# roysubhankar/dwt-domain-adaptation

Measured on AMD Instinct MI355X. Metric: imgs_per_sec, higher is better.
Workload: dtype bf16; 1 GPU; model=resnet50-dwt-mec-3stream, global_batch=1536, seq_len=224, parallelism=dp1, per_domain_batch=512, group_size=4, whiten_mode=zca

## Files before the change

### dwt_amd/kernels/dispatch.py

```python
from __future__ import annotations

import os
import warnings

_ext = None
_tried = False


def _load():
    global _ext, _tried
    if _tried:
        return _ext
    _tried = True
    try:
        import glob
        import importlib.util
        import os.path as osp

        here = osp.dirname(__file__)
        sos = sorted(glob.glob(osp.join(here, "_dwt_hip*.so")))
        if sos:
            spec = importlib.util.spec_from_file_location("dwt_amd.kernels._dwt_hip", sos[0])
            mod = importlib.util.module_from_spec(spec)
            spec.loader.exec_module(mod)
            mod.set_norm_wide(os.environ.get("DWT_AMD_NORM_WIDE", "1") != "0")
            mod.set_dense_glds(os.environ.get("DWT_AMD_DENSE_GLDS", "1") != "0")
            _ext = mod
    except Exception as exc:
        warnings.warn(f"dwt_amd HIP extension failed to load: {exc}")
        _ext = None
    return _ext


def available() -> bool:
    import torch
    if not torch.cuda.is_available():
        return False
    return _load() is not None


def ext():
    e = _load()
    if e is None:
        raise RuntimeError(
            "dwt_amd HIP extension is not built. Run `python -m dwt_amd.kernels.build` "
            "(or the repo's __graft_entry__.build()) to compile it for gfx950."
        )
    return e


def require_or_warn(opname: str) -> None:
    if os.environ.get("DWT_AMD_ALLOW_EAGER") == "1":
        warnings.warn(f"dwt_amd: running {opname} in eager fallback (DWT_AMD_ALLOW_EAGER=1)")
        return
    raise RuntimeError(
        f"dwt_amd: op '{opname}' called on a GPU but the HIP extension is not "
        "loaded. Build it with `python -m dwt_amd.kernels.build`, or set "
        "DWT_AMD_ALLOW_EAGER=1 to debug with the eager path."
    )



def whiten_multi(x, gamma, beta, running_means, running_vars, cfg,
                 stats_acc=None):
    from . import hip_ops
    return hip_ops.whiten_multi(x, gamma, beta, running_means, running_vars,
                                cfg, stats_acc)


def batch_norm_multi(x, gamma, beta, running_means, running_vars, cfg,
                     stats_acc=None):
    from . import hip_ops
    return hip_ops.batch_norm_multi(x, gamma, beta, running_means,
                                    running_vars, cfg, stats_acc)


def mec_loss(x, y):
    from . import hip_ops
    return hip_ops.mec_loss(x, y)


def entropy_loss(x):
    from . import hip_ops
    return hip_ops.entropy_loss(x)


def ce_loss(x, target):
    from . import hip_ops
    return hip_ops.ce_loss(x, target)
```

### dwt_amd/kernels/hip_ops.py

```python
from __future__ import annotations

import warnings
import torch

from . import dispatch
from ..ops.functional import _dist_world

_GEN_G_MAX = 32
_warned = set()


def _whiten_layout(x, c, g):
    if x.dim() == 4 and x.is_contiguous(memory_format=torch.channels_last) \
            and not x.is_contiguous():
        if whiten_cl_supported(c, g):
            return "cl"
    return "nchw"


def whiten_cl_supported(c, g):
    if c % 64 == 0 and (c <= 256 or c % 256 == 0) and g in (2, 4):
        gw = min(c, 256) // g
        return gw > 0 and 256 % gw == 0
    return False


def bn_cl_supported(c):
    if c % 4 != 0 or (c > 1024 and c % 1024 != 0):
        return False
    nch = min(c, 1024) // 4
    return 256 % nch == 0


def _bn_layout(x, c):
    if x.dim() == 2 and x.is_contiguous() and bn_cl_supported(c):
        return "cl"
    if x.dim() == 4 and x.is_contiguous(memory_format=torch.channels_last) \
            and not x.is_contiguous() and bn_cl_supported(c):
        return "cl"
    return "nchw"


def _flat_affine(gamma, beta, c, like):
    if gamma is None:
        return False, torch.empty(0, device=like.device, dtype=like.dtype), \
            torch.empty(0, device=like.device, dtype=like.dtype)
    return True, gamma.detach().reshape(c).contiguous(), \
        beta.detach().reshape(c).contiguous()


def _ema_update(ext, rm, new_mean, rv, new_var, momentum):
    if rm.dtype == torch.float32 and rm.is_contiguous() \
            and rv.dtype == torch.float32 and rv.is_contiguous():
        ext.ema_update(rm, new_mean, rv, new_var, momentum)
    else:
        rm.mul_(1.0 - momentum).add_(
            new_mean.reshape(rm.shape).to(rm.dtype), alpha=momentum)
        rv.mul_(1.0 - momentum).add_(
            new_var.reshape(rv.shape).to(rv.dtype), alpha=momentum)


def _warn_once(key, msg):
    if key not in _warned:
        _warned.add(key)
        warnings.warn(msg)


def _allreduce(t):
    import torch.distributed as dist
    dist.all_reduce(t)
    return t


def _ext():
    return dispatch.ext()


def _f32c(t):
    return t.detach().to(torch.float32).contiguous()


def _usable_stats_acc(acc, x, layout, training, numel):
    if acc is None or not training or layout != "cl" or x.dim() != 4:
        return None
    if acc.dtype != torch.float32 or acc.device != x.device \
            or acc.numel() != numel or not acc.is_contiguous():
        return None
    return acc.detach().reshape(-1)


class _HipWhitenMulti(torch.autograd.Function):

    @staticmethod
    def forward(ctx, x, gamma, beta, running_means, running_vars, cfg,
                stats_acc=None, res=None):
        ext = _ext()
        parts = cfg["parts"]
        g = x.shape[1] // cfg["num_groups"]
        eps, momentum = cfg["eps"], cfg["momentum"]
        training, mode, relu = cfg["training"], cfg["mode"], cfg["relu"]
        track = cfg.get("track_running_stats", True)
        ns_iters = cfg.get("ns_iters", 7)
        use_batch = training or not track

        c = x.shape[1]
        layout = _whiten_layout(x, c, g)
        if layout == "nchw":
            x = x.contiguous()
        n, c, h, w = x.shape
        assert n % parts == 0,             f"batch {n} not divisible by {parts} domain branches"
        b = n // parts
        n_groups = c // g
        ng_all = parts * n_groups
        dev = x.device
        m_count = b * h * w

        has_affine, gflat, bflat = _flat_affine(gamma, beta, c, x)

        world = _dist_world()[1] if cfg.get("stats_sync") and use_batch else 1
        ctx_count = m_count * world

        out = torch.empty_like(x)
        if use_batch:
            acc = _usable_stats_acc(stats_acc, x, layout, training,
                                    ng_all * (g + g * g))
            if acc is None:
                acc = torch.zeros(ng_all * (g + g * g), device=dev, dtype=torch.float32)
                if layout == "cl":
                    ext.whiten_stats_partial_cl(x, acc, g, c, m_count, parts)
                else:
                    ext.whiten_stats_partial(x, acc, g, parts)
            if world > 1:
                _allreduce(acc)
            mean = torch.empty(parts * c, device=dev, dtype=torch.float32)
            cov = torch.empty(ng_all, g, g, device=dev, dtype=torch.float32)
            ext.whiten_stats_final(acc, mean, cov, g, ng_all, ctx_count)
        else:
            mean = torch.stack([_f32c(running_means[p]).reshape(c)
                                for p in range(parts)]).reshape(-1).contiguous()
            cov = torch.stack([_f32c(running_vars[p]).reshape(n_groups, g, g)
                               for p in range(parts)]).reshape(ng_all, g, g).contiguous()

        wmat = torch.empty(ng_all, g, g, device=dev, dtype=torch.float32)
        if mode == "chol":
            ell = torch.empty_like(wmat)
            ext.matfn_chol_fwd(cov, wmat, ell, eps)
            saved_mat = ell
        else:
            ys = torch.empty(ng_all, ns_iters, g, g, device=dev, dtype=torch.float32)
            zs = torch.empty_like(ys)
            svals = torch.empty(ng_all, device=dev, dtype=torch.float32)
            ext.matfn_ns_fwd(cov, wmat, ys, zs, svals, eps, ns_iters)
            saved_mat = (ys, zs, svals)

        if res is not None:
            assert layout == "cl"
            ext.whiten_apply_res_cl(x, mean, wmat, gflat, bflat, res, out, g,
                                    c, m_count, True, has_affine, parts)
        elif layout == "cl":
            ext.whiten_apply_cl(x, mean, wmat, gflat, bflat, out, g, c,
                                m_count, relu, has_affine, parts)
        else:
            ext.whiten_apply(x, mean, wmat, gflat, bflat, out, g, relu,
                             has_affine, parts)

        if training and track and running_means is not None:
            with torch.no_grad():
                for p in range(parts):
                    _ema_update(ext, running_means[p], mean[p * c:(p + 1) * c],
                                running_vars[p],
                                cov[p * n_groups:(p + 1) * n_groups], momentum)

        ctx.cfg = cfg
        ctx.g = g
        ctx.layout = layout
        ctx.m_count = ctx_count
        ctx.m_local = m_count
        ctx.sync_world = world
        ctx.mean = mean
        ctx.wmat = wmat
        ctx.saved_mat = saved_mat
        ctx.has_affine = has_affine
        ctx.gflat = gflat
        ctx.bflat = bflat
        ctx.save_for_backward(x, gamma, out)
        return out

    @staticmethod
    def backward(ctx, dout):
        dx, _, dgamma, dbeta = _HipWhitenMulti.run_backward(ctx, dout)
        return dx, dgamma, dbeta, None, None, None, None

    @staticmethod
    def run_backward(ctx, dout, gb=None, join=False):
        ext = _ext()
        cfg = ctx.cfg
        parts, relu, mode, eps = cfg["parts"], cfg["relu"], cfg["mode"], cfg["eps"]
        training = cfg["training"]
        track = cfg.get("track_running_stats", True)
        ns_iters = cfg.get("ns_iters", 7)
        use_batch = training or not track
        g = ctx.g
        x, gamma, out = ctx.saved_tensors
        c = x.shape[1]
        ng_all = parts * (c // g)
        dev = x.device
        layout = ctx.layout
        if layout == "cl":
            dout = dout.contiguous(memory_format=torch.channels_last)
        else:
            dout = dout.contiguous()
        mean, wmat = ctx.mean, ctx.wmat
        m_count = ctx.m_count
        m_local = ctx.m_local

        dgb = torch.zeros(parts, 2, c, device=dev, dtype=torch.float32)
        dW = torch.zeros(ng_all, g, g, device=dev, dtype=torch.float32)
        dx = torch.empty_like(x)

        gid = None
        if join:
            assert layout == "cl"
            if gb is not None:
                gb = gb.contiguous(memory_format=torch.channels_last)
            gid = torch.empty_like(x)
            ext.whiten_join_bwd_reduce_cl(x, out, dout, gb, mean, wmat,
                                          ctx.gflat, gid, dW, dgb.reshape(-1),
                                          g, c, m_local, ctx.has_affine, parts)
            dout, relu = gid, False
        elif layout == "cl":
            ext.whiten_bwd_reduce_cl(x, dout, mean, wmat, ctx.gflat, ctx.bflat,
                                     dW, dgb.reshape(-1), g, c, m_local,
                                     relu, ctx.has_affine, parts)
        else:
            ext.whiten_bwd_reduce(x, dout, out, mean, wmat, ctx.gflat, dW,
                                  dgb.reshape(-1), g, relu, ctx.has_affine,
                                  parts)

        if use_batch:
            gdb = (ctx.gflat.float().unsqueeze(0) * dgb[:, 1]) if ctx.has_affine \
                else dgb[:, 1]
            gdb = gdb.reshape(-1).contiguous()
            dW_in = dW
            if ctx.sync_world > 1:
                dW_in = _allreduce(dW.clone())
                gdb = _allreduce(gdb.clone())
            S = torch.empty(ng_all, g, g, device=dev, dtype=torch.float32)
            corr = torch.empty(parts * c, device=dev, dtype=torch.float32)
            inv_m = 1.0 / m_count
            if mode == "chol":
                ext.matfn_chol_bwd(dW_in, wmat, ctx.saved_mat, gdb, S, corr,
                                   eps, inv_m)
            else:
                ys, zs, svals = ctx.saved_mat
                ext.matfn_ns_bwd(dW_in, wmat, ys, zs, svals, gdb, S, corr,
                                 eps, inv_m, ns_iters)
        else:
            S = torch.empty(0, device=dev)
            corr = torch.empty(0, device=dev)

        if layout == "cl":
            ext.whiten_bwd_apply_cl(x, dout, mean, wmat, ctx.gflat, ctx.bflat,
                                    S, corr, dx, g, c, m_local, relu,
                                    ctx.has_affine, use_batch, parts)
        else:
            ext.whiten_bwd_apply(x, dout, out, mean, wmat, ctx.gflat, S, corr,
                                 dx, g, relu, ctx.has_affine, use_batch, parts)

        if ctx.has_affine:
            dgamma = dgb[:, 0].sum(0).reshape(gamma.shape).to(gamma.dtype)
            dbeta = dgb[:, 1].sum(0).reshape(gamma.shape).to(gamma.dtype)
        else:
            dgamma = dbeta = None
        return dx, gid, dgamma, dbeta


def join_supported(kind, x, identity, cfg):
    if x.dtype not in (torch.float32, torch.bfloat16) or x.dim() != 4:
        return False
    if identity.shape != x.shape or identity.dtype != x.dtype \
            or identity.device != x.device \
            or identity.stride() != x.stride():
        return False
    c = x.shape[1]
    if kind == "whiten":
        return _whiten_layout(x, c, c // cfg["num_groups"]) == "cl"
    return _bn_layout(x, c) == "cl"


def whiten_join(x, identity, gamma, beta, running_means, running_vars, cfg,
                stats_acc=None):
    return _HipWhitenJoin.apply(x, identity, gamma, beta, running_means,
                                running_vars, cfg, stats_acc)


def batch_norm_join(x, identity, gamma, beta, running_means, running_vars, cfg,
                    stats_acc=None):
    return _HipBatchNormJoin.apply(x, identity, gamma, beta, running_means,
                                   running_vars, cfg, stats_acc)


def whiten_multi(x, gamma, beta, running_means, running_vars, cfg,
                 stats_acc=None):
    g = x.shape[1] // cfg["num_groups"]
    if g > _GEN_G_MAX or x.dtype not in (torch.float32, torch.bfloat16):
        _warn_once(("wh", g, x.dtype),
                   f"dwt_amd: whiten_multi g={g} dtype={x.dtype} uses the "
                   "torch path (HIP kernels cover g <= 32, fp32/bf16)")
        from ..ops.functional import WhitenMulti
        return WhitenMulti.apply(x, gamma, beta, running_means, running_vars, cfg)
    return _HipWhitenMulti.apply(x, gamma, beta, running_means, running_vars,
                                 cfg, stats_acc)


class _HipBatchNormMulti(torch.autograd.Function):
    @staticmethod
    def forward(ctx, x, gamma, beta, running_means, running_vars, cfg,
                stats_acc=None, res=None):
        ext = _ext()
        parts = cfg["parts"]
        eps, momentum = cfg["eps"], cfg["momentum"]
        training, relu = cfg["training"], cfg["relu"]
        track = cfg.get("track_running_stats", True)
        use_batch = training or not track

        spatial = x.dim() == 4
        c = x.shape[1]
        layout = _bn_layout(x, c)
        if layout == "nchw" or x.dim() == 2:
            x = x.contiguous()
        n = x.shape[0]
        assert n % parts == 0,             f"batch {n} not divisible by {parts} domain branches"
        dev = x.device
        cnt = (x.numel() // parts) // c

        has_affine, gflat, bflat = _flat_affine(gamma, beta, c, x)

        world = _dist_world()[1] if cfg.get("stats_sync") and use_batch else 1
        cnt_total = cnt * world

        out = torch.empty_like(x)
        if use_batch:
            acc = _usable_stats_acc(stats_acc, x, layout, training,
                                    parts * 2 * c)
            if acc is None:
                acc = torch.zeros(parts * 2 * c, device=dev, dtype=torch.float32)
                if layout == "cl":
                    ext.bn_stats_partial_cl(x, acc, c, cnt, parts)
                else:
                    ext.bn_stats_partial(x, acc, parts)
            if world > 1:
                _allreduce(acc)
            mean = torch.empty(parts * c, device=dev, dtype=torch.float32)
            istd = torch.empty(parts * c, device=dev, dtype=torch.float32)
            var_unb = torch.empty(parts * c, device=dev, dtype=torch.float32)
            ext.bn_stats_final(acc, mean, istd, var_unb, c, parts, cnt_total,
                               eps)
            if training and track and running_means is not None:
                with torch.no_grad():
                    for p in range(parts):
                        _ema_update(ext, running_means[p],
                                    mean[p * c:(p + 1) * c], running_vars[p],
                                    var_unb[p * c:(p + 1) * c], momentum)
        else:
            mean = torch.stack([_f32c(running_means[p]).reshape(c)
                                for p in range(parts)]).reshape(-1).contiguous()
            var = torch.stack([_f32c(running_vars[p]).reshape(c)
                               for p in range(parts)]).reshape(-1)
            istd = torch.rsqrt(var + eps).contiguous()

        if res is not None:
            assert layout == "cl" and x.dim() == 4
            ext.bn_apply_res_cl(x, mean, istd, gflat, bflat, res, out, c, cnt,
                                True, has_affine, parts)
        elif layout == "cl":
            ext.bn_apply_cl(x, mean, istd, gflat, bflat, out, c, cnt, relu,
                            has_affine, parts)
        else:
            ext.bn_apply(x, mean, istd, gflat, bflat, out, relu, has_affine,
                         parts)

        ctx.cfg = cfg
        ctx.layout = layout
        ctx.cnt = cnt
        ctx.cnt_total = cnt_total
        ctx.sync_world = world
        ctx.spatial = spatial
        ctx.mean = mean
        ctx.istd = istd
        ctx.has_affine = has_affine
        ctx.gflat = gflat
        ctx.bflat = bflat
        ctx.use_batch = use_batch
        ctx.save_for_backward(x, gamma, out)
        return out

    @staticmethod
    def backward(ctx, dout):
        dx, _, dgamma, dbeta = _HipBatchNormMulti.run_backward(ctx, dout)
        return dx, dgamma, dbeta, None, None, None, None

    @staticmethod
    def run_backward(ctx, dout, gb=None, join=False):
        ext = _ext()
        cfg = ctx.cfg
        parts, relu = cfg["parts"], cfg["relu"]
        x, gamma, out = ctx.saved_tensors
        c = x.shape[1]
        dev = x.device
        layout = ctx.layout
        if layout == "cl" and x.dim() == 4:
            dout = dout.contiguous(memory_format=torch.channels_last)
        else:
            dout = dout.contiguous()
        mean, istd = ctx.mean, ctx.istd

        sums = torch.zeros(parts, 2, c, device=dev, dtype=torch.float32)
        dx = torch.empty_like(x)
        gid = None
        if join:
            assert layout == "cl"
            if gb is not None:
                gb = gb.contiguous(memory_format=torch.channels_last)
            gid = torch.empty_like(x)
            ext.bn_join_bwd_reduce_cl(x, out, dout, gb, mean, istd, gid,
                                      sums.reshape(-1), c, ctx.cnt, parts)
            dout, relu = gid, False
        elif layout == "cl":
            ext.bn_bwd_reduce_cl(x, dout, mean, istd, ctx.gflat, ctx.bflat,
                                 sums.reshape(-1), c, ctx.cnt, relu,
                                 ctx.has_affine, parts)
        else:
            ext.bn_bwd_reduce(x, dout, out, mean, istd, sums.reshape(-1), relu,
                              parts)

        apply_sums = sums.reshape(-1)
        if ctx.sync_world > 1:
            apply_sums = _allreduce(apply_sums.clone())
        if layout == "cl":
            ext.bn_bwd_apply_cl(x, dout, mean, istd, ctx.gflat, ctx.bflat,
                                apply_sums, dx, c, ctx.cnt, relu,
                                ctx.has_affine, ctx.use_batch, parts,
                                ctx.cnt_total)
        else:
            ext.bn_bwd_apply(x, dout, out, mean, istd, ctx.gflat, apply_sums,
                             dx, relu, ctx.has_affine, ctx.use_batch,
                             ctx.cnt_total, parts)

        if ctx.has_affine:
            dgamma = sums[:, 1].sum(0).reshape(gamma.shape).to(gamma.dtype)
            dbeta = sums[:, 0].sum(0).reshape(gamma.shape).to(gamma.dtype)
        else:
            dgamma = dbeta = None
        return dx, gid, dgamma, dbeta


def _join_function(name, site):

    def forward(ctx, x, identity, gamma, beta, running_means, running_vars,
                cfg, stats_acc=None):
        ctx.set_materialize_grads(False)
        res = identity.detach()
        y = site.forward(ctx, x, gamma, beta, running_means, running_vars,
                         cfg, stats_acc, res=res)
        return y, y.view_as(y)

    def backward(ctx, ga, gb):
        if ga is None and gb is None:
            return (None,) * 8
        if ga is None:
            ga, gb = gb, None
        dx, gid, dgamma, dbeta = site.run_backward(ctx, ga, gb, join=True)
        return dx, gid, dgamma, dbeta, None, None, None, None

    return type(name, (torch.autograd.Function,),
                {"__doc__": _join_function.__doc__,
                 "forward": staticmethod(forward),
                 "backward": staticmethod(backward)})


_HipWhitenJoin = _join_function("_HipWhitenJoin", _HipWhitenMulti)
_HipBatchNormJoin = _join_function("_HipBatchNormJoin", _HipBatchNormMulti)


def batch_norm_multi(x, gamma, beta, running_means, running_vars, cfg,
                     stats_acc=None):
    if x.dtype not in (torch.float32, torch.bfloat16):
        from ..ops.functional import BatchNormMulti
        return BatchNormMulti.apply(x, gamma, beta, running_means, running_vars, cfg)
    return _HipBatchNormMulti.apply(x, gamma, beta, running_means, running_vars,
                                    cfg, stats_acc)


class _HipMecLoss(torch.autograd.Function):
    @staticmethod
    def forward(ctx, x, y):
        ext = _ext()
        x32 = x.detach().to(torch.float32).contiguous()
        y32 = y.detach().to(torch.float32).contiguous()
        n, k = x32.shape
        lx = torch.empty_like(x32)
        ly = torch.empty_like(y32)
        amin = torch.empty(n, device=x.device, dtype=torch.int32)
        loss = torch.zeros(1, device=x.device, dtype=torch.float32)
        ext.mec_fwd(x32, y32, lx, ly, amin, loss)
        ctx.save_for_backward(lx, ly, amin)
        ctx.dtypes = (x.dtype, y.dtype)
        return loss[0]

    @staticmethod
    def backward(ctx, dloss):
        ext = _ext()
        lx, ly, amin = ctx.saved_tensors
        gscale = dloss.detach().to(torch.float32).reshape(1).contiguous()
        dx = torch.empty_like(lx)
        dy = torch.empty_like(ly)
        ext.mec_bwd(lx, ly, amin, gscale, dx, dy)
        return dx.to(ctx.dtypes[0]), dy.to(ctx.dtypes[1])


class _HipEntropyLoss(torch.autograd.Function):
    @staticmethod
    def forward(ctx, x):
        ext = _ext()
        x32 = x.detach().to(torch.float32).contiguous()
        n, k = x32.shape
        q = torch.empty_like(x32)
        hper = torch.empty(n, device=x.device, dtype=torch.float32)
        loss = torch.zeros(1, device=x.device, dtype=torch.float32)
        ext.entropy_fwd(x32, q, hper, loss)
        ctx.save_for_backward(q, hper)
        ctx.dtype = x.dtype
        return loss[0]

    @staticmethod
    def backward(ctx, dloss):
        ext = _ext()
        q, hper = ctx.saved_tensors
        gscale = dloss.detach().to(torch.float32).reshape(1).contiguous()
        dx = torch.empty_like(q)
        ext.entropy_bwd(q, hper, gscale, dx)
        return dx.to(ctx.dtype)


def mec_loss(x, y):
    return _HipMecLoss.apply(x, y)


def entropy_loss(x):
    return _HipEntropyLoss.apply(x)


class _HipCELoss(torch.autograd.Function):

    @staticmethod
    def forward(ctx, x, target):
        ext = _ext()
        x32 = x.detach().to(torch.float32).contiguous()
        q = torch.empty_like(x32)
        loss = torch.zeros(1, device=x.device, dtype=torch.float32)
        ext.ce_fwd(x32, target.contiguous(), q, loss)
        ctx.save_for_backward(q, target)
        ctx.dtype = x.dtype
        return loss[0]

    @staticmethod
    def backward(ctx, dloss):
        ext = _ext()
        q, target = ctx.saved_tensors
        gscale = dloss.detach().to(torch.float32).reshape(1).contiguous()
        dx = torch.empty_like(q)
        ext.ce_bwd(q, target.contiguous(), gscale, dx)
        return dx.to(ctx.dtype), None


def ce_loss(x, target):
    return _HipCELoss.apply(x, target)
```

### dwt_amd/kernels/src/dwt_kernels.hip

```cpp

#include <torch/extension.h>
#include <ATen/cuda/CUDAContext.h>
#include <hip/hip_runtime.h>

#include <cstdint>
#include <initializer_list>
#include <string>
#include <type_traits>
#include <vector>

#define DEV_INLINE __device__ __forceinline__

namespace dwt {


DEV_INLINE float ldf(const float* p) { return *p; }
DEV_INLINE float ldf(const c10::BFloat16* p) {
  unsigned short u = *reinterpret_cast<const unsigned short*>(p);
  union { unsigned int i; float f; } v;
  v.i = static_cast<unsigned int>(u) << 16;
  return v.f;
}
DEV_INLINE void stf(float* p, float v) { *p = v; }
DEV_INLINE void stf(c10::BFloat16* p, float v) {
  union { unsigned int i; float f; } u;
  u.f = v;
  unsigned int lsb = (u.i >> 16) & 1u;
  unsigned int rounded = u.i + 0x7fffu + lsb;
  *reinterpret_cast<unsigned short*>(p) = static_cast<unsigned short>(rounded >> 16);
}

template <typename T> struct VecTraits;
template <> struct VecTraits<float> {
  static constexpr int W = 4;
  DEV_INLINE static void load(const float* p, float* out) {
    const float4 v = *reinterpret_cast<const float4*>(p);
    out[0] = v.x; out[1] = v.y; out[2] = v.z; out[3] = v.w;
  }
  DEV_INLINE static void store(float* p, const float* in) {
    *reinterpret_cast<float4*>(p) = make_float4(in[0], in[1], in[2], in[3]);
  }
};
template <> struct VecTraits<c10::BFloat16> {
  static constexpr int W = 8;
  DEV_INLINE static void load(const c10::BFloat16* p, float* out) {
    const uint4 v = *reinterpret_cast<const uint4*>(p);
    const unsigned int w[4] = {v.x, v.y, v.z, v.w};
#pragma unroll
    for (int i = 0; i < 4; ++i) {
      union { unsigned int u; float f; } lo, hi;
      lo.u = (w[i] & 0xffffu) << 16;
      hi.u = w[i] & 0xffff0000u;
      out[2 * i] = lo.f;
      out[2 * i + 1] = hi.f;
    }
  }
  DEV_INLINE static void store(c10::BFloat16* p, const float* in) {
    unsigned int w[4];
#pragma unroll
    for (int i = 0; i < 4; ++i) {
      union { unsigned int u; float f; } a, b;
      a.f = in[2 * i]; b.f = in[2 * i + 1];
      unsigned int la = (a.u >> 16) & 1u, lb = (b.u >> 16) & 1u;
      unsigned int ra = (a.u + 0x7fffu + la) >> 16;
      unsigned int rb = (b.u + 0x7fffu + lb) >> 16;
      w[i] = (ra & 0xffffu) | (rb << 16);
    }
    *reinterpret_cast<uint4*>(p) = make_uint4(w[0], w[1], w[2], w[3]);
  }
};

DEV_INLINE float wave_reduce_sum(float v) {
#pragma unroll
  for (int off = 32; off > 0; off >>= 1) v += __shfl_down(v, off, 64);
  return v;
}

template <int NV, typename IdxFn>
DEV_INLINE void block_reduce_atomic(float (&vals)[NV], float* lds,
                                    float* gout, IdxFn idx) {
  const int lane = threadIdx.x & 63;
  const int wid = threadIdx.x >> 6;
  const int nwaves = blockDim.x >> 6;
#pragma unroll
  for (int k = 0; k < NV; ++k) {
    const float r = wave_reduce_sum(vals[k]);
    if (lane == 0) lds[wid * NV + k] = r;
  }
  __syncthreads();
  for (int k = threadIdx.x; k < NV; k += blockDim.x) {
    float acc = 0.f;
    for (int w = 0; w < nwaves; ++w) acc += lds[w * NV + k];
    atomicAdd(&gout[idx(k)], acc);
  }
  __syncthreads();
}


template <typename T, int G, bool VECTOR>
__global__ void whiten_stats_partial_kernel(
    const T* __restrict__ x, float* __restrict__ acc,
    int B, int C, int64_t HW, int64_t M) {
  constexpr int VW = VECTOR ? VecTraits<T>::W : 1;
  const int grp = blockIdx.y;
  const int c0 = grp * G;
  float s[G];
  float p[G][G];
#pragma unroll
  for (int i = 0; i < G; ++i) {
    s[i] = 0.f;
#pragma unroll
    for (int j = 0; j < G; ++j) p[i][j] = 0.f;
  }
  const int64_t nvec = M / VW;
  const int64_t stride = (int64_t)gridDim.x * blockDim.x;
  for (int64_t mv = (int64_t)blockIdx.x * blockDim.x + threadIdx.x; mv < nvec; mv += stride) {
    const int64_t el = mv * VW;
    const int64_t n = el / HW, hw = el - n * HW;
    const T* base = x + ((n * C + c0) * HW + hw);
    float v[G][VW];
#pragma unroll
    for (int j = 0; j < G; ++j) {
      if (VECTOR) VecTraits<T>::load(base + (int64_t)j * HW, v[j]);
      else v[j][0] = ldf(base + (int64_t)j * HW);
    }
#pragma unroll
    for (int k = 0; k < VW; ++k) {
#pragma unroll
      for (int i = 0; i < G; ++i) {
        s[i] += v[i][k];
#pragma unroll
        for (int j = 0; j <= i; ++j) p[i][j] += v[i][k] * v[j][k];
      }
    }
  }
  float* gacc = acc + (int64_t)grp * (G + G * G);
  constexpr int NTRI = G * (G + 1) / 2;
  __shared__ float red_lds[4 * (G + NTRI)];
  float vals[G + NTRI];
#pragma unroll
  for (int i = 0; i < G; ++i) vals[i] = s[i];
#pragma unroll
  for (int i = 0; i < G; ++i)
#pragma unroll
    for (int j = 0; j <= i; ++j) vals[G + i * (i + 1) / 2 + j] = p[i][j];
  block_reduce_atomic<G + NTRI>(vals, red_lds, gacc, [](int k) {
    if (k < G) return k;
    int kk = k - G, i = 0;
    while (kk > i) { kk -= (i + 1); ++i; }
    return G + i * G + kk;
  });
}

__global__ void whiten_stats_final_kernel(
    const float* __restrict__ acc, float* __restrict__ mean,
    float* __restrict__ cov, int n_groups, int g, float inv_m) {
  const int grp = blockIdx.x;
  const int i = threadIdx.x / g, j = threadIdx.x % g;
  if (i >= g) return;
  const float* gacc = acc + (int64_t)grp * (g + g * g);
  const float mi = gacc[i] * inv_m;
  const float mj = gacc[j] * inv_m;
  const float pij = (j <= i) ? gacc[g + i * g + j] : gacc[g + j * g + i];
  cov[((int64_t)grp * g + i) * g + j] = pij * inv_m - mi * mj;
  if (j == 0) mean[grp * g + i] = mi;
}


#define GEN_MT 64

template <typename T>
DEV_INLINE void gen_load_tile(const T* __restrict__ x, float* tile, int g,
                              int C, int64_t HW, int64_t m0, int64_t M,
                              const float* __restrict__ sub ) {
  for (int idx = threadIdx.x; idx < g * GEN_MT; idx += blockDim.x) {
    const int c = idx / GEN_MT;
    const int ml = idx % GEN_MT;
    const int64_t m = m0 + ml;
    float v = 0.f;
    if (m < M) {
      const int64_t n = m / HW, hw = m - n * HW;
      v = ldf(x + (n * C + c) * HW + hw);
      if (sub) v -= sub[c];
    }
    tile[c * (GEN_MT + 1) + ml] = v;
  }
}

template <typename T>
__global__ void whiten_stats_gen_kernel(
    const T* __restrict__ x, float* __restrict__ acc,
    int g, int C, int64_t HW, int64_t M) {
  __shared__ float tile[32 * (GEN_MT + 1)];
  const int grp = blockIdx.y;
  const int c0 = grp * g;
  const int ntri = g * (g + 1) / 2;
  float p[3] = {0.f, 0.f, 0.f};
  float s = 0.f;
  const int64_t stride = (int64_t)gridDim.x * GEN_MT;
  for (int64_t m0 = (int64_t)blockIdx.x * GEN_MT; m0 < M; m0 += stride) {
    gen_load_tile(x + (int64_t)c0 * HW, tile, g, C, HW, m0, M, nullptr);
    __syncthreads();
    for (int pi = 0; pi < 3; ++pi) {
      const int pr = threadIdx.x + pi * 256;
      if (pr >= ntri) break;
      int i = 0, kk = pr;
      while (kk > i) { kk -= (i + 1); ++i; }
      const float* ri = tile + i * (GEN_MT + 1);
      const float* rj = tile + kk * (GEN_MT + 1);
      float a = 0.f;
#pragma unroll 4
      for (int ml = 0; ml < GEN_MT; ++ml) a += ri[ml] * rj[ml];
      p[pi] += a;
    }
    if (threadIdx.x < (unsigned)g) {
      const float* ri = tile + threadIdx.x * (GEN_MT + 1);
      float a = 0.f;
#pragma unroll 4
      for (int ml = 0; ml < GEN_MT; ++ml) a += ri[ml];
      s += a;
    }
    __syncthreads();
  }
  float* gacc = acc + (int64_t)grp * (g + g * g);
  if (threadIdx.x < (unsigned)g) atomicAdd(&gacc[threadIdx.x], s);
  for (int pi = 0; pi < 3; ++pi) {
    const int pr = threadIdx.x + pi * 256;
    if (pr >= ntri) break;
    int i = 0, kk = pr;
    while (kk > i) { kk -= (i + 1); ++i; }
    atomicAdd(&gacc[g + i * g + kk], p[pi]);
  }
}

template <typename T>
__global__ void whiten_apply_gen_kernel(
    const T* __restrict__ x, const float* __restrict__ mean,
    const float* __restrict__ W, const T* __restrict__ gamma,
    const T* __restrict__ beta, T* __restrict__ out,
    int g, int C, int64_t HW, int64_t M, int relu, int has_affine) {
  __shared__ float tile[32 * (GEN_MT + 1)];
  __shared__ float Ws[32 * 32];
  __shared__ float ms[32], gs[32], bs[32];
  const int grp = blockIdx.y;
  const int c0 = grp * g;
  for (int e = threadIdx.x; e < g * g; e += blockDim.x)
    Ws[e] = W[(int64_t)grp * g * g + e];
  if (threadIdx.x < (unsigned)g) {
    ms[threadIdx.x] = mean[c0 + threadIdx.x];
    gs[threadIdx.x] = has_affine ? ldf(gamma + c0 + threadIdx.x) : 1.f;
    bs[threadIdx.x] = has_affine ? ldf(beta + c0 + threadIdx.x) : 0.f;
  }
  __syncthreads();
  const int64_t stride = (int64_t)gridDim.x * GEN_MT;
  const int ml = threadIdx.x % GEN_MT;
  const int cstep = blockDim.x / GEN_MT;
  for (int64_t m0 = (int64_t)blockIdx.x * GEN_MT; m0 < M; m0 += stride) {
    gen_load_tile(x + (int64_t)c0 * HW, tile, g, C, HW, m0, M, ms);
    __syncthreads();
    const int64_t m = m0 + ml;
    if (m < M) {
      const int64_t n = m / HW, hw = m - n * HW;
      for (int c = threadIdx.x / GEN_MT; c < g; c += cstep) {
        float a = 0.f;
        for (int j = 0; j < g; ++j)
          a += Ws[c * g + j] * tile[j * (GEN_MT + 1) + ml];
        a = a * gs[c] + bs[c];
        if (relu) a = fmaxf(a, 0.f);
        stf(out + ((int64_t)n * C + c0 + c) * HW + hw, a);
      }
    }
    __syncthreads();
  }
}

template <typename T>
DEV_INLINE void gen_load_dy(const T* __restrict__ dout, const T* __restrict__ outp,
                            float* tile, int g, int C, int64_t HW, int64_t m0,
                            int64_t M, int relu) {
  for (int idx = threadIdx.x; idx < g * GEN_MT; idx += blockDim.x) {
    const int c = idx / GEN_MT;
    const int ml = idx % GEN_MT;
    const int64_t m = m0 + ml;
    float v = 0.f;
    if (m < M) {
      const int64_t n = m / HW, hw = m - n * HW;
      const int64_t off = (n * C + c) * HW + hw;
      v = ldf(dout + off);
      if (relu && ldf(outp + off) <= 0.f) v = 0.f;
    }
    tile[c * (GEN_MT + 1) + ml] = v;
  }
}

template <typename T>
__global__ void whiten_bwd_reduce_gen_kernel(
    const T* __restrict__ x, const T* __restrict__ dout,
    const T* __restrict__ outp, const float* __restrict__ mean,
    const float* __restrict__ W, const T* __restrict__ gamma,
    float* __restrict__ dWacc, float* __restrict__ dgb,
    int g, int C, int64_t HW, int64_t M, int relu, int has_affine) {
  __shared__ float xt[32 * (GEN_MT + 1)];
  __shared__ float dyt[32 * (GEN_MT + 1)];
  __shared__ float ms[32];
  const int grp = blockIdx.y;
  const int c0 = grp * g;
  if (threadIdx.x < (unsigned)g) ms[threadIdx.x] = mean[c0 + threadIdx.x];
  __syncthreads();
  const int npair = g * g;
  float p[4] = {0.f, 0.f, 0.f, 0.f};
  float db = 0.f;
  const int64_t stride = (int64_t)gridDim.x * GEN_MT;
  const int64_t xoff = (int64_t)c0 * HW;
  for (int64_t m0 = (int64_t)blockIdx.x * GEN_MT; m0 < M; m0 += stride) {
    gen_load_tile(x + xoff, xt, g, C, HW, m0, M, ms);
    gen_load_dy(dout + xoff, outp + xoff, dyt, g, C, HW, m0, M, relu);
    __syncthreads();
    for (int pi = 0; pi < 4; ++pi) {
      const int pr = threadIdx.x + pi * 256;
      if (pr >= npair) break;
      const int i = pr / g, j = pr % g;
      const float* ri = dyt + i * (GEN_MT + 1);
      const float* rj = xt + j * (GEN_MT + 1);
      float a = 0.f;
#pragma unroll 4
      for (int ml = 0; ml < GEN_MT; ++ml) a += ri[ml] * rj[ml];
      p[pi] += a;
    }
    if (threadIdx.x < (unsigned)g) {
      const float* ri = dyt + threadIdx.x * (GEN_MT + 1);
      float a = 0.f;
#pragma unroll 4
      for (int ml = 0; ml < GEN_MT; ++ml) a += ri[ml];
      db += a;
    }
    __syncthreads();
  }
  if (threadIdx.x < (unsigned)g)
    atomicAdd(&dgb[C + c0 + threadIdx.x], db);
  for (int pi = 0; pi < 4; ++pi) {
    const int pr = threadIdx.x + pi * 256;
    if (pr >= npair) break;
    const int i = pr / g, j = pr % g;
    const float gm = has_affine ? ldf(gamma + c0 + i) : 1.f;
    atomicAdd(&dWacc[(int64_t)grp * g * g + pr], gm * p[pi]);
    atomicAdd(&dgb[c0 + i], W[(int64_t)grp * g * g + i * g + j] * p[pi]);
  }
}

template <typename T>
__global__ void whiten_bwd_apply_gen_kernel(
    const T* __restrict__ x, const T* __restrict__ dout,
    const T* __restrict__ outp, const float* __restrict__ mean,
    const float* __restrict__ W, const T* __restrict__ gamma,
    const float* __restrict__ S, const float* __restrict__ corr,
    T* __restrict__ dx, int g, int C, int64_t HW, int64_t M, int relu,
    int has_affine, int train_stats) {
  __shared__ float xt[32 * (GEN_MT + 1)];
  __shared__ float dyt[32 * (GEN_MT + 1)];
  __shared__ float Ws[32 * 32];
  __shared__ float Ss[32 * 32];
  __shared__ float ms[32], gs[32], cr[32];
  const int grp = blockIdx.y;
  const int c0 = grp * g;
  for (int e = threadIdx.x; e < g * g; e += blockDim.x) {
    Ws[e] = W[(int64_t)grp * g * g + e];
    Ss[e] = train_stats ? S[(int64_t)grp * g * g + e] : 0.f;
  }
  if (threadIdx.x < (unsigned)g) {
    ms[threadIdx.x] = mean[c0 + threadIdx.x];
    gs[threadIdx.x] = has_affine ? ldf(gamma + c0 + threadIdx.x) : 1.f;
    cr[threadIdx.x] = train_stats ? corr[c0 + threadIdx.x] : 0.f;
  }
  __syncthreads();
  const int64_t stride = (int64_t)gridDim.x * GEN_MT;
  const int ml = threadIdx.x % GEN_MT;
  const int cstep = blockDim.x / GEN_MT;
  const int64_t xoff = (int64_t)c0 * HW;
  for (int64_t m0 = (int64_t)blockIdx.x * GEN_MT; m0 < M; m0 += stride) {
    gen_load_tile(x + xoff, xt, g, C, HW, m0, M, ms);
    gen_load_dy(dout + xoff, outp + xoff, dyt, g, C, HW, m0, M, relu);
    __syncthreads();
    const int64_t m = m0 + ml;
    if (m < M) {
      const int64_t n = m / HW, hw = m - n * HW;
      for (int c = threadIdx.x / GEN_MT; c < g; c += cstep) {
        float a = -cr[c];
        for (int j = 0; j < g; ++j)
          a += Ws[j * g + c] * gs[j] * dyt[j * (GEN_MT + 1) + ml] +
               Ss[c * g + j] * xt[j * (GEN_MT + 1) + ml];
        stf(dx + ((int64_t)n * C + c0 + c) * HW + hw, a);
      }
    }
    __syncthreads();
  }
}


#define MATFN_MAX_G 32

__global__ void matfn_chol_fwd_kernel(
    const float* __restrict__ cov, float* __restrict__ Wout,
    float* __restrict__ Lout, int g, float eps) {
  __shared__ float A[MATFN_MAX_G * MATFN_MAX_G];
  __shared__ float Wl[MATFN_MAX_G * MATFN_MAX_G];
  const int grp = blockIdx.x;
  const int t = threadIdx.x;
  const int64_t base = (int64_t)grp * g * g;
  for (int e = t; e < g * g; e += 64) {
    const int i = e / g, j = e % g;
    A[e] = (1.f - eps) * cov[base + e] + (i == j ? eps : 0.f);
  }
  __syncthreads();
  for (int k = 0; k < g; ++k) {
    if (t == 0) A[k * g + k] = sqrtf(A[k * g + k]);
    __syncthreads();
    const float dk = A[k * g + k];
    for (int i = k + 1 + t; i < g; i += 64) A[i * g + k] /= dk;
    __syncthreads();
    for (int e = t; e < (g - k - 1) * (g - k - 1); e += 64) {
      const int jj = k + 1 + e / (g - k - 1);
      const int ii = k + 1 + e % (g - k - 1);
      if (ii >= jj) A[ii * g + jj] -= A[ii * g + k] * A[jj * g + k];
    }
    __syncthreads();
  }
  for (int c = t; c < g; c += 64) {
    for (int i = 0; i < g; ++i) {
      float v = (i == c) ? 1.f : 0.f;
      for (int j = c; j < i; ++j) v -= A[i * g + j] * Wl[j * g + c];
      Wl[i * g + c] = (i >= c) ? v / A[i * g + i] : 0.f;
    }
  }
  __syncthreads();
  for (int e = t; e < g * g; e += 64) {
    const int i = e / g, j = e % g;
    Wout[base + e] = Wl[e];
    Lout[base + e] = (i >= j) ? A[e] : 0.f;
  }
}

__global__ void matfn_chol_bwd_kernel(
    const float* __restrict__ dW, const float* __restrict__ W,
    const float* __restrict__ L, const float* __restrict__ gdb,
    float* __restrict__ S, float* __restrict__ corr,
    int g, float eps, float inv_m) {
  __shared__ float sW[MATFN_MAX_G * MATFN_MAX_G];
  __shared__ float t0[MATFN_MAX_G * MATFN_MAX_G];
  __shared__ float t1[MATFN_MAX_G * MATFN_MAX_G];
  const int grp = blockIdx.x;
  const int t = threadIdx.x;
  const int64_t base = (int64_t)grp * g * g;
  for (int e = t; e < g * g; e += 64) { sW[e] = W[base + e]; t0[e] = dW[base + e]; }
  __syncthreads();
  for (int e = t; e < g * g; e += 64) {
    const int i = e / g, j = e % g;
    float v = 0.f;
    for (int k = 0; k < g; ++k) v += sW[k * g + i] * t0[k * g + j];
    t1[e] = v;
  }
  __syncthreads();
  for (int e = t; e < g * g; e += 64) {
    const int i = e / g, j = e % g;
    float v = 0.f;
    for (int k = 0; k < g; ++k) v += t1[i * g + k] * sW[j * g + k];
    t0[e] = (i >= j) ? -v : 0.f;
  }
  __syncthreads();
  for (int e = t; e < g * g; e += 64) {
    const int i = e / g, j = e % g;
    float v = 0.f;
    for (int k = 0; k < g; ++k) v += L[base + k * g + i] * t0[k * g + j];
    t1[e] = (i > j) ? v : (i == j ? 0.5f * v : 0.f);
  }
  __syncthreads();
  for (int e = t; e < g * g; e += 64) {
    const int i = e / g, j = e % g;
    float v = 0.f;
    for (int k = 0; k < g; ++k) v += sW[k * g + i] * t1[k * g + j];
    t0[e] = v;
  }
  __syncthreads();
  for (int e = t; e < g * g; e += 64) {
    const int i = e / g, j = e % g;
    float v = 0.f;
    for (int k = 0; k < g; ++k) v += t0[i * g + k] * sW[k * g + j];
    t1[e] = v;
  }
  __syncthreads();
  const float sc = (1.f - eps) * inv_m;
  for (int e = t; e < g * g; e += 64) {
    const int i = e / g, j = e % g;
    S[base + e] = sc * (t1[i * g + j] + t1[j * g + i]);
  }
  for (int i = t; i < g; i += 64) {
    float v = 0.f;
    for (int j = 0; j < g; ++j) v += sW[j * g + i] * gdb[grp * g + j];
    corr[grp * g + i] = v * inv_m;
  }
}

__global__ void matfn_ns_fwd_kernel(
    const float* __restrict__ cov, float* __restrict__ Wout,
    float* __restrict__ ys, float* __restrict__ zs, float* __restrict__ svals,
    int g, float eps, int iters) {
  __shared__ float Y[MATFN_MAX_G * MATFN_MAX_G];
  __shared__ float Z[MATFN_MAX_G * MATFN_MAX_G];
  __shared__ float Tm[MATFN_MAX_G * MATFN_MAX_G];
  __shared__ float NY[MATFN_MAX_G * MATFN_MAX_G];
  __shared__ float NZ[MATFN_MAX_G * MATFN_MAX_G];
  __shared__ float s_sh;
  const int grp = blockIdx.x;
  const int t = threadIdx.x;
  const int64_t base = (int64_t)grp * g * g;
  for (int e = t; e < g * g; e += 64) {
    const int i = e / g, j = e % g;
    Y[e] = (1.f - eps) * cov[base + e] + (i == j ? eps : 0.f);
  }
  __syncthreads();
  if (t == 0) {
    float tr = 0.f;
    for (int i = 0; i < g; ++i) tr += Y[i * g + i];
    s_sh = fmaxf(tr, 1e-30f);
    svals[grp] = s_sh;
  }
  __syncthreads();
  const float s = s_sh;
  for (int e = t; e < g * g; e += 64) {
    Y[e] /= s;
    Z[e] = (e / g == e % g) ? 1.f : 0.f;
  }
  __syncthreads();
  for (int it = 0; it < iters; ++it) {
    float* ysave = ys + ((int64_t)grp * iters + it) * g * g;
    float* zsave = zs + ((int64_t)grp * iters + it) * g * g;
    for (int e = t; e < g * g; e += 64) {
      ysave[e] = Y[e];
      zsave[e] = Z[e];
      const int i = e / g, j = e % g;
      float v = 0.f;
      for (int k = 0; k < g; ++k) v += Z[i * g + k] * Y[k * g + j];
      Tm[e] = 0.5f * ((i == j ? 3.f : 0.f) - v);
    }
    __syncthreads();
    for (int e = t; e < g * g; e += 64) {
      const int i = e / g, j = e % g;
      float vy = 0.f, vz = 0.f;
      for (int k = 0; k < g; ++k) {
        vy += Y[i * g + k] * Tm[k * g + j];
        vz += Tm[i * g + k] * Z[k * g + j];
      }
      NY[e] = vy;
      NZ[e] = vz;
    }
    __syncthreads();
    for (int e = t; e < g * g; e += 64) { Y[e] = NY[e]; Z[e] = NZ[e]; }
    __syncthreads();
  }
  const float inv_sqrt_s = rsqrtf(s);
  for (int e = t; e < g * g; e += 64) Wout[base + e] = Z[e] * inv_sqrt_s;
}

__global__ void matfn_ns_bwd_kernel(
    const float* __restrict__ dW, const float* __restrict__ W,
    const float* __restrict__ ys, const float* __restrict__ zs,
    const float* __restrict__ svals, const float* __restrict__ gdb,
    float* __restrict__ S, float* __restrict__ corr,
    int g, float eps, float inv_m, int iters) {
  __shared__ float YB[MATFN_MAX_G * MATFN_MAX_G];
  __shared__ float ZB[MATFN_MAX_G * MATFN_MAX_G];
  __shared__ float Tm[MATFN_MAX_G * MATFN_MAX_G];
  __shared__ float TB[MATFN_MAX_G * MATFN_MAX_G];
  __shared__ float NY[MATFN_MAX_G * MATFN_MAX_G];
  __shared__ float NZ[MATFN_MAX_G * MATFN_MAX_G];
  __shared__ float red[1];
  const int grp = blockIdx.x;
  const int t = threadIdx.x;
  const int64_t base = (int64_t)grp * g * g;
  const float s = svals[grp];
  const float inv_sqrt_s = rsqrtf(s);

  float sbar_part = 0.f;
  for (int e = t; e < g * g; e += 64) {
    const float d = dW[base + e];
    ZB[e] = d * inv_sqrt_s;
    YB[e] = 0.f;
    sbar_part += d * W[base + e];
  }
  sbar_part = wave_reduce_sum(sbar_part);
  if (t == 0) red[0] = sbar_part * (-0.5f) / s;
  __syncthreads();
  float sbar = red[0];

  for (int it = iters - 1; it >= 0; --it) {
    const float* y = ys + ((int64_t)grp * iters + it) * g * g;
    const float* z = zs + ((int64_t)grp * iters + it) * g * g;
    for (int e = t; e < g * g; e += 64) {
      const int i = e / g, j = e % g;
      float v = 0.f;
      for (int k = 0; k < g; ++k) v += z[i * g + k] * y[k * g + j];
      Tm[e] = 0.5f * ((i == j ? 3.f : 0.f) - v);
    }
    __syncthreads();
    for (int e = t; e < g * g; e += 64) {
      const int i = e / g, j = e % g;
      float v = 0.f;
      for (int k = 0; k < g; ++k)
        v += y[k * g + i] * YB[k * g + j] + ZB[i * g + k] * z[j * g + k];
      TB[e] = v;
    }
    __syncthreads();
    for (int e = t; e < g * g; e += 64) {
      const int i = e / g, j = e % g;
      float vy = 0.f, vz = 0.f;
      for (int k = 0; k < g; ++k) {
        vy += YB[i * g + k] * Tm[j * g + k] - 0.5f * z[k * g + i] * TB[k * g + j];
        vz += Tm[k * g + i] * ZB[k * g + j] - 0.5f * TB[i * g + k] * y[j * g + k];
      }
      NY[e] = vy;
      NZ[e] = vz;
    }
    __syncthreads();
    for (int e = t; e < g * g; e += 64) { YB[e] = NY[e]; ZB[e] = NZ[e]; }
    __syncthreads();
  }

  const float* y0 = ys + (int64_t)grp * iters * g * g;
  float dot = 0.f;
  for (int e = t; e < g * g; e += 64) dot += YB[e] * y0[e];
  dot = wave_reduce_sum(dot);
  if (t == 0) red[0] = dot;
  __syncthreads();
  sbar -= red[0] / s;

  const float sc = (1.f - eps) * inv_m;
  for (int e = t; e < g * g; e += 64) {
    const int i = e / g, j = e % g;
    const float raw_ij = YB[i * g + j] / s + (i == j ? sbar : 0.f);
    const float raw_ji = YB[j * g + i] / s + (i == j ? sbar : 0.f);
    S[base + e] = sc * (raw_ij + raw_ji);
  }
  for (int i = t; i < g; i += 64) {
    float v = 0.f;
    for (int j = 0; j < g; ++j) v += W[base + j * g + i] * gdb[grp * g + j];
    corr[grp * g + i] = v * inv_m;
  }
}


template <typename T, int G, bool VECTOR>
__global__ void whiten_apply_kernel(
    const T* __restrict__ x, const float* __restrict__ mean,
    const float* __restrict__ W, const T* __restrict__ gamma,
    const T* __restrict__ beta, T* __restrict__ out,
    int C, int64_t HW, int relu, int has_affine) {
  constexpr int VW = VECTOR ? VecTraits<T>::W : 1;
  const int grp = blockIdx.z;
  const int n = blockIdx.y;
  const int c0 = grp * G;
  const int64_t hw0 = ((int64_t)blockIdx.x * blockDim.x + threadIdx.x) * VW;
  if (hw0 >= HW) return;

  float m[G], Wr[G][G], gm[G], bt[G];
#pragma unroll
  for (int i = 0; i < G; ++i) {
    m[i] = mean[c0 + i];
    gm[i] = has_affine ? ldf(gamma + c0 + i) : 1.f;
    bt[i] = has_affine ? ldf(beta + c0 + i) : 0.f;
#pragma unroll
    for (int j = 0; j < G; ++j) Wr[i][j] = W[((int64_t)grp * G + i) * G + j];
  }

  const T* xb = x + ((int64_t)n * C + c0) * HW + hw0;
  T* ob = out + ((int64_t)n * C + c0) * HW + hw0;
  float xv[G][VW];
  if (VECTOR) {
#pragma unroll
    for (int j = 0; j < G; ++j) VecTraits<T>::load(xb + (int64_t)j * HW, xv[j]);
  } else {
#pragma unroll
    for (int j = 0; j < G; ++j) xv[j][0] = ldf(xb + (int64_t)j * HW);
  }
#pragma unroll
  for (int j = 0; j < G; ++j)
#pragma unroll
    for (int v = 0; v < VW; ++v) xv[j][v] -= m[j];

#pragma unroll
  for (int i = 0; i < G; ++i) {
    float yv[VW];
#pragma unroll
    for (int v = 0; v < VW; ++v) {
      float a = 0.f;
#pragma unroll
      for (int j = 0; j < G; ++j) a += Wr[i][j] * xv[j][v];
      a = a * gm[i] + bt[i];
      yv[v] = relu ? fmaxf(a, 0.f) : a;
    }
    if (VECTOR) VecTraits<T>::store(ob + (int64_t)i * HW, yv);
    else stf(ob + (int64_t)i * HW, yv[0]);
  }
}


template <typename T, int G, bool VECTOR>
__global__ void whiten_bwd_reduce_kernel(
    const T* __restrict__ x, const T* __restrict__ dout,
    const T* __restrict__ out, const float* __restrict__ mean,
    const float* __restrict__ W, const T* __restrict__ gamma,
    float* __restrict__ dWacc, float* __restrict__ dgb,
    int B, int C, int64_t HW, int64_t M, int relu, int has_affine) {
  constexpr int VW = VECTOR ? VecTraits<T>::W : 1;
  const int grp = blockIdx.y;
  const int c0 = grp * G;
  float m[G], Wr[G][G], gm[G];
#pragma unroll
  for (int i = 0; i < G; ++i) {
    m[i] = mean[c0 + i];
    gm[i] = has_affine ? ldf(gamma + c0 + i) : 1.f;
#pragma unroll
    for (int j = 0; j < G; ++j) Wr[i][j] = W[((int64_t)grp * G + i) * G + j];
  }
  float dWl[G][G], dg[G], db[G];
#pragma unroll
  for (int i = 0; i < G; ++i) {
    dg[i] = 0.f; db[i] = 0.f;
#pragma unroll
    for (int j = 0; j < G; ++j) dWl[i][j] = 0.f;
  }

  const int64_t nvec = M / VW;
  const int64_t stride = (int64_t)gridDim.x * blockDim.x;
  for (int64_t mv = (int64_t)blockIdx.x * blockDim.x + threadIdx.x; mv < nvec; mv += stride) {
    const int64_t el = mv * VW;
    const int64_t n = el / HW, hw = el - n * HW;
    const int64_t off = ((int64_t)n * C + c0) * HW + hw;
    float xv[G][VW], dyv[G][VW];
#pragma unroll
    for (int j = 0; j < G; ++j) {
      if (VECTOR) {
        VecTraits<T>::load(x + off + (int64_t)j * HW, xv[j]);
        VecTraits<T>::load(dout + off + (int64_t)j * HW, dyv[j]);
        if (relu) {
          float ov[VW];
          VecTraits<T>::load(out + off + (int64_t)j * HW, ov);
#pragma unroll
          for (int v = 0; v < VW; ++v) dyv[j][v] = ov[v] > 0.f ? dyv[j][v] : 0.f;
        }
      } else {
        xv[j][0] = ldf(x + off + (int64_t)j * HW);
        float d = ldf(dout + off + (int64_t)j * HW);
        if (relu) d = ldf(out + off + (int64_t)j * HW) > 0.f ? d : 0.f;
        dyv[j][0] = d;
      }
#pragma unroll
      for (int v = 0; v < VW; ++v) xv[j][v] -= m[j];
    }
#pragma unroll
    for (int v = 0; v < VW; ++v) {
#pragma unroll
      for (int i = 0; i < G; ++i) {
        const float dy = dyv[i][v];
        db[i] += dy;
        float y0 = 0.f;
#pragma unroll
        for (int j = 0; j < G; ++j) y0 += Wr[i][j] * xv[j][v];
        dg[i] += dy * y0;
        const float dy0 = dy * gm[i];
#pragma unroll
        for (int j = 0; j < G; ++j) dWl[i][j] += dy0 * xv[j][v];
      }
    }
  }

  float* gdW = dWacc + (int64_t)grp * G * G;
  __shared__ float red_lds[4 * G * G];
  {
    float vals[2 * G];
#pragma unroll
    for (int i = 0; i < G; ++i) { vals[i] = dg[i]; vals[G + i] = db[i]; }
    block_reduce_atomic<2 * G>(vals, red_lds, dgb, [c0, C](int k) {
      return k < G ? c0 + k : C + c0 + (k - G);
    });
  }
  {
    float vals[G * G];
#pragma unroll
    for (int i = 0; i < G; ++i)
#pragma unroll
      for (int j = 0; j < G; ++j) vals[i * G + j] = dWl[i][j];
    block_reduce_atomic<G * G>(vals, red_lds, gdW, [](int k) { return k; });
  }
}


template <typename T, int G, bool VECTOR>
__global__ void whiten_bwd_apply_kernel(
    const T* __restrict__ x, const T* __restrict__ dout,
    const T* __restrict__ out, const float* __restrict__ mean,
// ... 578 lines not shown
#pragma unroll
  for (int k = 0; k < VC; ++k) {
    atomicAdd(&lacc[cb + k], a[k]);
    atomicAdd(&lacc[L.CW + cb + k], b[k]);
  }
  __syncthreads();
  for (int k = threadIdx.x; k < L.CW; k += blockDim.x) {
    atomicAdd(&acc[blockIdx.z * 1024 + k], lacc[k]);
    atomicAdd(&acc[C + blockIdx.z * 1024 + k], lacc[L.CW + k]);
  }
}

template <typename T, int VC, int R>
__global__ void bn_stats_nhwc_kernel(
    const T* __restrict__ x, float* __restrict__ acc, int C, int64_t M) {
  const int part = blockIdx.y;
  x += (int64_t)part * M * C;
  acc += (int64_t)part * 2 * C;
  const BnLanes<VC> L(C);
  float s[VC], ss[VC];
#pragma unroll
  for (int k = 0; k < VC; ++k) { s[k] = 0.f; ss[k] = 0.f; }
  for_rows<R>(L, M, [&](int64_t m, int64_t stride, auto n) {
    constexpr int N = decltype(n)::value;
    float v[N][VC];
#pragma unroll
    for (int r = 0; r < N; ++r)
      load_group<T, VC>(x + (m + r * stride) * C + L.c0, v[r]);
#pragma unroll
    for (int r = 0; r < N; ++r)
#pragma unroll
      for (int k = 0; k < VC; ++k) { s[k] += v[r][k]; ss[k] += v[r][k] * v[r][k]; }
  });
  bn_two_sum_flush(L, C, s, ss, acc);
}

template <typename T, int VC, int R, bool RES>
__global__ void bn_apply_nhwc_kernel(
    const T* __restrict__ x, const T* __restrict__ res,
    const float* __restrict__ mean,
    const float* __restrict__ istd, const T* __restrict__ gamma,
    const T* __restrict__ beta, T* __restrict__ out, int C, int64_t M,
    int relu, int has_affine) {
  const int part = blockIdx.y;
  x += (int64_t)part * M * C;
  if constexpr (RES) res += (int64_t)part * M * C;
  out += (int64_t)part * M * C;
  mean += (int64_t)part * C;
  istd += (int64_t)part * C;
  const BnLanes<VC> L(C);
  float mu[VC], is[VC], gm[VC], bt[VC];
#pragma unroll
  for (int k = 0; k < VC; ++k) {
    mu[k] = mean[L.c0 + k];
    is[k] = istd[L.c0 + k];
    gm[k] = has_affine ? ldf(gamma + L.c0 + k) : 1.f;
    bt[k] = has_affine ? ldf(beta + L.c0 + k) : 0.f;
  }
  for_rows<R>(L, M, [&](int64_t m, int64_t stride, auto n) {
    constexpr int N = decltype(n)::value;
    [[maybe_unused]] float r[N][VC];
    float v[N][VC];
#pragma unroll
    for (int i = 0; i < N; ++i) {
      load_group<T, VC>(x + (m + i * stride) * C + L.c0, v[i]);
      if constexpr (RES) load_group<T, VC>(res + (m + i * stride) * C + L.c0, r[i]);
    }
#pragma unroll
    for (int i = 0; i < N; ++i) {
#pragma unroll
      for (int k = 0; k < VC; ++k) {
        float y = (v[i][k] - mu[k]) * is[k] * gm[k] + bt[k];
        if constexpr (RES) y += r[i][k];
        v[i][k] = relu ? fmaxf(y, 0.f) : y;
      }
      store_group<T, VC>(out + (m + i * stride) * C + L.c0, v[i]);
    }
  });
}

template <typename T, int VC, int R, bool JOIN>
__global__ void bn_bwd_reduce_nhwc_kernel(
    const T* __restrict__ x, const T* __restrict__ dout,
    const T* __restrict__ y, const T* __restrict__ gb, T* __restrict__ gid,
    const float* __restrict__ mean,
    const float* __restrict__ istd, const T* __restrict__ gamma,
    const T* __restrict__ beta, float* __restrict__ sums, int C,
    int64_t M, int relu, int has_affine) {
  const int part = blockIdx.y;
  const int64_t poff = (int64_t)part * M * C;
  x += poff; dout += poff;
  if constexpr (JOIN) {
    y += poff; gid += poff;
    if (gb) gb += poff;
  }
  mean += (int64_t)part * C;
  istd += (int64_t)part * C;
  sums += (int64_t)part * 2 * C;
  const BnLanes<VC> L(C);
  float mu[VC], is[VC], gm[VC], bt[VC];
#pragma unroll
  for (int k = 0; k < VC; ++k) {
    mu[k] = mean[L.c0 + k];
    is[k] = istd[L.c0 + k];
    gm[k] = has_affine ? ldf(gamma + L.c0 + k) : 1.f;
    bt[k] = has_affine ? ldf(beta + L.c0 + k) : 0.f;
  }
  float s_dy[VC], s_dyxh[VC];
#pragma unroll
  for (int k = 0; k < VC; ++k) { s_dy[k] = 0.f; s_dyxh[k] = 0.f; }
  for_rows<R>(L, M, [&](int64_t m, int64_t stride, auto n) {
    constexpr int N = decltype(n)::value;
    [[maybe_unused]] float yv[N][VC];
    float xv[N][VC], dv[N][VC];
#pragma unroll
    for (int i = 0; i < N; ++i) {
      if constexpr (JOIN) {
        const int64_t off = (m + i * stride) * C + L.c0;
        load_group<T, VC>(x + off, xv[i]);
        load_group<T, VC>(y + off, yv[i]);
        join_sum<T, VC>(dout, gb, off, dv[i]);
      } else {
        load_group<T, VC>(x + (m + i * stride) * C + L.c0, xv[i]);
        load_group<T, VC>(dout + (m + i * stride) * C + L.c0, dv[i]);
      }
    }
#pragma unroll
    for (int i = 0; i < N; ++i) {
#pragma unroll
      for (int k = 0; k < VC; ++k) {
        if constexpr (JOIN)
          dv[i][k] = yv[i][k] > 0.f ? round_to<T>(dv[i][k]) : 0.f;
        const float xh = (xv[i][k] - mu[k]) * is[k];
        if constexpr (!JOIN) {
          if (relu && gm[k] * xh + bt[k] <= 0.f) dv[i][k] = 0.f;
        }
        s_dy[k] += dv[i][k];
        s_dyxh[k] += dv[i][k] * xh;
      }
      if constexpr (JOIN)
        store_group<T, VC>(gid + (m + i * stride) * C + L.c0, dv[i]);
    }
  });
  bn_two_sum_flush(L, C, s_dy, s_dyxh, sums);
}

template <typename T, int VC, int R>
__global__ void bn_bwd_apply_nhwc_kernel(
    const T* __restrict__ x, const T* __restrict__ dout,
    const float* __restrict__ mean,
    const float* __restrict__ istd, const T* __restrict__ gamma,
    const T* __restrict__ beta,
    const float* __restrict__ sums, T* __restrict__ dx, int C, int64_t M,
    float inv_m, int relu, int has_affine, int use_batch) {
  const int part = blockIdx.y;
  const int64_t poff = (int64_t)part * M * C;
  x += poff; dout += poff; dx += poff;
  mean += (int64_t)part * C;
  istd += (int64_t)part * C;
  sums += (int64_t)part * 2 * C;
  const BnLanes<VC> L(C);
  float mu[VC], is[VC], gm[VC], bt[VC], mdy[VC], mdyxh[VC];
#pragma unroll
  for (int k = 0; k < VC; ++k) {
    const int c = L.c0 + k;
    mu[k] = mean[c];
    is[k] = istd[c];
    gm[k] = has_affine ? ldf(gamma + c) : 1.f;
    bt[k] = has_affine ? ldf(beta + c) : 0.f;
    mdy[k] = use_batch ? sums[c] * inv_m : 0.f;
    mdyxh[k] = use_batch ? sums[C + c] * inv_m : 0.f;
  }
  for_rows<R>(L, M, [&](int64_t m, int64_t stride, auto n) {
    constexpr int N = decltype(n)::value;
    float xv[N][VC], dv[N][VC];
#pragma unroll
    for (int i = 0; i < N; ++i) {
      load_group<T, VC>(x + (m + i * stride) * C + L.c0, xv[i]);
      load_group<T, VC>(dout + (m + i * stride) * C + L.c0, dv[i]);
    }
#pragma unroll
    for (int i = 0; i < N; ++i) {
#pragma unroll
      for (int k = 0; k < VC; ++k) {
        const float xh = (xv[i][k] - mu[k]) * is[k];
        if (relu && gm[k] * xh + bt[k] <= 0.f) dv[i][k] = 0.f;
        const float dxh = dv[i][k] * gm[k];
        if (use_batch) {
          dv[i][k] = (dxh - gm[k] * mdy[k] - xh * gm[k] * mdyxh[k]) * is[k];
        } else {
          dv[i][k] = dxh * is[k];
        }
      }
      store_group<T, VC>(dx + (m + i * stride) * C + L.c0, dv[i]);
    }
  });
}


template <typename T, bool VECTOR>
__global__ void bn_stats_partial_kernel(
    const T* __restrict__ x, float* __restrict__ acc,
    int B, int C, int64_t HW, int64_t M) {
  constexpr int VW = VECTOR ? VecTraits<T>::W : 1;
  const int c = blockIdx.y;
  float s = 0.f, ss = 0.f;
  const int64_t nvec = M / VW;
  const int64_t stride = (int64_t)gridDim.x * blockDim.x;
  for (int64_t mv = (int64_t)blockIdx.x * blockDim.x + threadIdx.x; mv < nvec; mv += stride) {
    const int64_t el = mv * VW;
    const int64_t n = el / HW, hw = el - n * HW;
    const T* p = x + ((int64_t)n * C + c) * HW + hw;
    if (VECTOR) {
      float v[VW];
      VecTraits<T>::load(p, v);
#pragma unroll
      for (int k = 0; k < VW; ++k) { s += v[k]; ss += v[k] * v[k]; }
    } else {
      const float v = ldf(p);
      s += v; ss += v * v;
    }
  }
  __shared__ float red_lds[4 * 2];
  float vals[2] = {s, ss};
  block_reduce_atomic<2>(vals, red_lds, acc, [c, C](int k) {
    return k == 0 ? c : C + c;
  });
}

__global__ void bn_stats_final_kernel(
    const float* __restrict__ acc, float* __restrict__ mean,
    float* __restrict__ istd, float* __restrict__ var_unb,
    int total, int Cper, float inv_m, float unb_scale, float eps) {
  const int i = blockIdx.x * blockDim.x + threadIdx.x;
  if (i >= total) return;
  const int p = i / Cper, c = i % Cper;
  const int64_t base = (int64_t)p * 2 * Cper;
  const float mu = acc[base + c] * inv_m;
  float var = fmaxf(acc[base + Cper + c] * inv_m - mu * mu, 0.f);
  mean[i] = mu;
  istd[i] = rsqrtf(var + eps);
  var_unb[i] = var * unb_scale;
}

template <typename T, bool VECTOR>
__global__ void bn_apply_kernel(
    const T* __restrict__ x, const float* __restrict__ mean,
    const float* __restrict__ istd, const T* __restrict__ gamma,
    const T* __restrict__ beta, T* __restrict__ out,
    int C, int64_t HW, int relu, int has_affine) {
  constexpr int VW = VECTOR ? VecTraits<T>::W : 1;
  const int c = blockIdx.z;
  const int n = blockIdx.y;
  const int64_t hw0 = ((int64_t)blockIdx.x * blockDim.x + threadIdx.x) * VW;
  if (hw0 >= HW) return;
  const float mu = mean[c], is = istd[c];
  const float gm = has_affine ? ldf(gamma + c) : 1.f;
  const float bt = has_affine ? ldf(beta + c) : 0.f;
  const int64_t off = ((int64_t)n * C + c) * HW + hw0;
  float v[VW];
  if (VECTOR) VecTraits<T>::load(x + off, v);
  else v[0] = ldf(x + off);
#pragma unroll
  for (int k = 0; k < VW; ++k) {
    float y = (v[k] - mu) * is * gm + bt;
    v[k] = relu ? fmaxf(y, 0.f) : y;
  }
  if (VECTOR) VecTraits<T>::store(out + off, v);
  else stf(out + off, v[0]);
}

template <typename T, bool VECTOR>
__global__ void bn_bwd_reduce_kernel(
    const T* __restrict__ x, const T* __restrict__ dout,
    const T* __restrict__ out, const float* __restrict__ mean,
    const float* __restrict__ istd, float* __restrict__ sums,
    int B, int C, int64_t HW, int64_t M, int relu) {
  constexpr int VW = VECTOR ? VecTraits<T>::W : 1;
  const int c = blockIdx.y;
  const float mu = mean[c], is = istd[c];
  float s_dy = 0.f, s_dyxh = 0.f;
  const int64_t nvec = M / VW;
  const int64_t stride = (int64_t)gridDim.x * blockDim.x;
  for (int64_t mv = (int64_t)blockIdx.x * blockDim.x + threadIdx.x; mv < nvec; mv += stride) {
    const int64_t el = mv * VW;
    const int64_t n = el / HW, hw = el - n * HW;
    const int64_t off = ((int64_t)n * C + c) * HW + hw;
    float xv[VW], dv[VW];
    if (VECTOR) {
      VecTraits<T>::load(x + off, xv);
      VecTraits<T>::load(dout + off, dv);
      if (relu) {
        float ov[VW];
        VecTraits<T>::load(out + off, ov);
#pragma unroll
        for (int k = 0; k < VW; ++k) dv[k] = ov[k] > 0.f ? dv[k] : 0.f;
      }
    } else {
      xv[0] = ldf(x + off);
      dv[0] = ldf(dout + off);
      if (relu) dv[0] = ldf(out + off) > 0.f ? dv[0] : 0.f;
    }
#pragma unroll
    for (int k = 0; k < VW; ++k) {
      s_dy += dv[k];
      s_dyxh += dv[k] * (xv[k] - mu) * is;
    }
  }
  __shared__ float red_lds[4 * 2];
  float vals[2] = {s_dy, s_dyxh};
  block_reduce_atomic<2>(vals, red_lds, sums, [c, C](int k) {
    return k == 0 ? c : C + c;
  });
}

template <typename T, bool VECTOR>
__global__ void bn_bwd_apply_kernel(
    const T* __restrict__ x, const T* __restrict__ dout,
    const T* __restrict__ out, const float* __restrict__ mean,
    const float* __restrict__ istd, const T* __restrict__ gamma,
    const float* __restrict__ sums, T* __restrict__ dx,
    int C, int64_t HW, float inv_m, int relu, int has_affine, int use_batch) {
  constexpr int VW = VECTOR ? VecTraits<T>::W : 1;
  const int c = blockIdx.z;
  const int n = blockIdx.y;
  const int64_t hw0 = ((int64_t)blockIdx.x * blockDim.x + threadIdx.x) * VW;
  if (hw0 >= HW) return;
  const float mu = mean[c], is = istd[c];
  const float gm = has_affine ? ldf(gamma + c) : 1.f;
  const float m_dy = sums[c] * inv_m;
  const float m_dyxh = sums[C + c] * inv_m;
  const int64_t off = ((int64_t)n * C + c) * HW + hw0;
  float xv[VW], dv[VW];
  if (VECTOR) {
    VecTraits<T>::load(x + off, xv);
    VecTraits<T>::load(dout + off, dv);
    if (relu) {
      float ov[VW];
      VecTraits<T>::load(out + off, ov);
#pragma unroll
      for (int k = 0; k < VW; ++k) dv[k] = ov[k] > 0.f ? dv[k] : 0.f;
    }
  } else {
    xv[0] = ldf(x + off);
    dv[0] = ldf(dout + off);
    if (relu) dv[0] = ldf(out + off) > 0.f ? dv[0] : 0.f;
  }
#pragma unroll
  for (int k = 0; k < VW; ++k) {
    const float dxh = dv[k] * gm;
    float r;
    if (use_batch) {
      const float xh = (xv[k] - mu) * is;
      r = (dxh - gm * m_dy - xh * gm * m_dyxh) * is;
    } else {
      r = dxh * is;
    }
    dv[k] = r;
  }
  if (VECTOR) VecTraits<T>::store(dx + off, dv);
  else stf(dx + off, dv[0]);
}


__global__ void ema_update_kernel(float* __restrict__ rm,
                                  const float* __restrict__ a, int64_t n1,
                                  float* __restrict__ rv,
                                  const float* __restrict__ b, int64_t n2,
                                  float momentum) {
  const int64_t i = (int64_t)blockIdx.x * blockDim.x + threadIdx.x;
  if (i < n1) {
    rm[i] = (1.f - momentum) * rm[i] + momentum * a[i];
  } else if (i < n1 + n2) {
    const int64_t j = i - n1;
    rv[j] = (1.f - momentum) * rv[j] + momentum * b[j];
  }
}


template <typename T>
__global__ void maxpool_nhwc_fwd_kernel(
    const T* __restrict__ x, T* __restrict__ out, uint8_t* __restrict__ idx,
    int C, int H, int W, int P, int Q, int KS, int stride, int pad,
    int64_t total) {
  const int64_t i = (int64_t)blockIdx.x * blockDim.x + threadIdx.x;
  if (i >= total) return;
  const int c = i % C;
  int64_t r = i / C;
  const int q = r % Q; r /= Q;
  const int p = r % P; r /= P;
  const int n = (int)r;
  float best = -INFINITY;
  int bidx = 0;
  for (int kh = 0; kh < KS; ++kh) {
    const int h = p * stride - pad + kh;
    if (h < 0 || h >= H) continue;
    for (int kw = 0; kw < KS; ++kw) {
      const int w = q * stride - pad + kw;
      if (w < 0 || w >= W) continue;
      const float v = ldf(x + (((int64_t)n * H + h) * W + w) * C + c);
      if (v > best) { best = v; bidx = kh * KS + kw; }
    }
  }
  stf(out + i, best);
  idx[i] = (uint8_t)bidx;
}

template <typename T>
__global__ void maxpool_nhwc_bwd_kernel(
    const T* __restrict__ dout, const uint8_t* __restrict__ idx,
    T* __restrict__ dx, int C, int H, int W, int P, int Q, int KS, int stride,
    int pad, int64_t total_in) {
  const int64_t i = (int64_t)blockIdx.x * blockDim.x + threadIdx.x;
  if (i >= total_in) return;
  const int c = i % C;
  int64_t r = i / C;
  const int w = r % W; r /= W;
  const int h = r % H; r /= H;
  const int n = (int)r;
  float acc = 0.f;
  const int pmin = max(0, (h + pad - KS + stride) / stride);
  const int pmax = min(P - 1, (h + pad) / stride);
  const int qmin = max(0, (w + pad - KS + stride) / stride);
  const int qmax = min(Q - 1, (w + pad) / stride);
  for (int p = pmin; p <= pmax; ++p) {
    const int kh = h - (p * stride - pad);
    if (kh < 0 || kh >= KS) continue;
    for (int q = qmin; q <= qmax; ++q) {
      const int kw = w - (q * stride - pad);
      if (kw < 0 || kw >= KS) continue;
      const int64_t o = (((int64_t)n * P + p) * Q + q) * C + c;
      if (idx[o] == (uint8_t)(kh * KS + kw)) acc += ldf(dout + o);
    }
  }
  stf(dx + i, acc);
}

template <typename T, int VC>
__global__ void maxpool_nhwc_fwd_vec_kernel(
    const T* __restrict__ x, T* __restrict__ out, uint8_t* __restrict__ idx,
    int C, int H, int W, int P, int Q, int KS, int stride, int pad,
    int64_t total_chunks) {
  const int64_t i = (int64_t)blockIdx.x * blockDim.x + threadIdx.x;
  if (i >= total_chunks) return;
  const int nc = C / VC;
  const int c0 = (int)(i % nc) * VC;
  int64_t r = i / nc;
  const int q = r % Q; r /= Q;
  const int p = r % P; r /= P;
  const int n = (int)r;
  float best[VC];
  uint8_t bidx[VC];
#pragma unroll
  for (int k = 0; k < VC; ++k) { best[k] = -INFINITY; bidx[k] = 0; }
  for (int kh = 0; kh < KS; ++kh) {
    const int h = p * stride - pad + kh;
    if (h < 0 || h >= H) continue;
    for (int kw = 0; kw < KS; ++kw) {
      const int w = q * stride - pad + kw;
      if (w < 0 || w >= W) continue;
      float v[VC];
      load_group<T, VC>(x + (((int64_t)n * H + h) * W + w) * C + c0, v);
      const uint8_t wi = (uint8_t)(kh * KS + kw);
#pragma unroll
      for (int k = 0; k < VC; ++k)
        if (v[k] > best[k]) { best[k] = v[k]; bidx[k] = wi; }
    }
  }
  const int64_t o = (((int64_t)n * P + p) * Q + q) * C + c0;
  store_group<T, VC>(out + o, best);
#pragma unroll
  for (int k = 0; k < VC; ++k) idx[o + k] = bidx[k];
}

template <typename T, int VC>
__global__ void maxpool_nhwc_bwd_vec_kernel(
    const T* __restrict__ dout, const uint8_t* __restrict__ idx,
    T* __restrict__ dx, int C, int H, int W, int P, int Q, int KS, int stride,
    int pad, int64_t total_chunks) {
  const int64_t i = (int64_t)blockIdx.x * blockDim.x + threadIdx.x;
  if (i >= total_chunks) return;
  const int nc = C / VC;
  const int c0 = (int)(i % nc) * VC;
  int64_t r = i / nc;
  const int w = r % W; r /= W;
  const int h = r % H; r /= H;
  const int n = (int)r;
  float acc[VC];
#pragma unroll
  for (int k = 0; k < VC; ++k) acc[k] = 0.f;
  const int pmin = max(0, (h + pad - KS + stride) / stride);
  const int pmax = min(P - 1, (h + pad) / stride);
  const int qmin = max(0, (w + pad - KS + stride) / stride);
  const int qmax = min(Q - 1, (w + pad) / stride);
  for (int p = pmin; p <= pmax; ++p) {
    const int kh = h - (p * stride - pad);
    if (kh < 0 || kh >= KS) continue;
    for (int q = qmin; q <= qmax; ++q) {
      const int kw = w - (q * stride - pad);
      if (kw < 0 || kw >= KS) continue;
      const int64_t o = (((int64_t)n * P + p) * Q + q) * C + c0;
      const uint8_t wi = (uint8_t)(kh * KS + kw);
      float dv[VC];
      load_group<T, VC>(dout + o, dv);
#pragma unroll
      for (int k = 0; k < VC; ++k)
        if (idx[o + k] == wi) acc[k] += dv[k];
    }
  }
  store_group<T, VC>(dx + (((int64_t)n * H + h) * W + w) * C + c0, acc);
}

template <typename T>
__global__ void gap_nhwc_fwd_kernel(const T* __restrict__ x,
                                    T* __restrict__ out, int C, int64_t HW,
                                    int N) {
  const int n = blockIdx.y;
  const int c = blockIdx.x * 64 + (threadIdx.x & 63);
  if (c >= C) return;
  const T* base = x + (int64_t)n * HW * C + c;
  float s = 0.f;
  for (int64_t m = 0; m < HW; ++m) s += ldf(base + m * C);
  stf(out + (int64_t)n * C + c, s / (float)HW);
}

template <typename T>
__global__ void gap_nhwc_bwd_kernel(const T* __restrict__ dout,
                                    T* __restrict__ dx, int C, int64_t HW,
// ... 151 lines not shown
}

__global__ void mec_bwd_kernel(
    const float* __restrict__ lx, const float* __restrict__ ly,
    const int* __restrict__ amin, const float* __restrict__ gscale,
    float* __restrict__ dx, float* __restrict__ dy, int N, int K) {
  const int64_t i = (int64_t)blockIdx.x * blockDim.x + threadIdx.x;
  if (i >= (int64_t)N * K) return;
  const int row = i / K, k = i % K;
  const float sc = gscale[0] / (2.f * N);
  const float oh = (k == amin[row]) ? 1.f : 0.f;
  dx[i] = (__expf(lx[i]) - oh) * sc;
  dy[i] = (__expf(ly[i]) - oh) * sc;
}

__global__ void entropy_fwd_kernel(
    const float* __restrict__ x, float* __restrict__ q,
    float* __restrict__ hper, float* __restrict__ loss, int N, int K) {
  const int row = blockIdx.x * (blockDim.x / 64) + (threadIdx.x / 64);
  const int lane = threadIdx.x & 63;
  if (row >= N) return;
  const float* xr = x + (int64_t)row * K;
  float mx = -INFINITY;
  for (int k = lane; k < K; k += 64) mx = fmaxf(mx, xr[k]);
#pragma unroll
  for (int off = 32; off > 0; off >>= 1) mx = fmaxf(mx, __shfl_down(mx, off, 64));
  mx = __shfl(mx, 0, 64);
  float s = 0.f;
  for (int k = lane; k < K; k += 64) s += __expf(xr[k] - mx);
  s = wave_reduce_sum(s);
  s = __shfl(s, 0, 64);
  const float lse = mx + __logf(s);
  float h = 0.f;
  for (int k = lane; k < K; k += 64) {
    const float qq = xr[k] - lse;
    q[(int64_t)row * K + k] = qq;
    h -= __expf(qq) * qq;
  }
  h = wave_reduce_sum(h);
  if (lane == 0) {
    hper[row] = h;
    atomicAdd(loss, h / N);
  }
}

__global__ void ce_fwd_kernel(
    const float* __restrict__ x, const int64_t* __restrict__ target,
    float* __restrict__ q, float* __restrict__ loss, int N, int K) {
  const int row = blockIdx.x * (blockDim.x / 64) + (threadIdx.x / 64);
  const int lane = threadIdx.x & 63;
  if (row >= N) return;
  const float* xr = x + (int64_t)row * K;
  float mx = -INFINITY;
  for (int k = lane; k < K; k += 64) mx = fmaxf(mx, xr[k]);
#pragma unroll
  for (int off = 32; off > 0; off >>= 1) mx = fmaxf(mx, __shfl_down(mx, off, 64));
  mx = __shfl(mx, 0, 64);
  float ssum = 0.f;
  for (int k = lane; k < K; k += 64) ssum += __expf(xr[k] - mx);
  ssum = wave_reduce_sum(ssum);
  ssum = __shfl(ssum, 0, 64);
  const float lse = mx + __logf(ssum);
  for (int k = lane; k < K; k += 64) q[(int64_t)row * K + k] = xr[k] - lse;
  if (lane == 0) atomicAdd(loss, (lse - xr[target[row]]) / N);
}

__global__ void ce_bwd_kernel(
    const float* __restrict__ q, const int64_t* __restrict__ target,
    const float* __restrict__ gscale, float* __restrict__ dx, int N, int K) {
  const int64_t i = (int64_t)blockIdx.x * blockDim.x + threadIdx.x;
  if (i >= (int64_t)N * K) return;
  const int row = i / K, k = i % K;
  const float oh = (k == (int)target[row]) ? 1.f : 0.f;
  dx[i] = (__expf(q[i]) - oh) * gscale[0] / N;
}

__global__ void entropy_bwd_kernel(
    const float* __restrict__ q, const float* __restrict__ hper,
    const float* __restrict__ gscale, float* __restrict__ dx, int N, int K) {
  const int64_t i = (int64_t)blockIdx.x * blockDim.x + threadIdx.x;
  if (i >= (int64_t)N * K) return;
  const int row = i / K;
  const float p = __expf(q[i]);
  dx[i] = -p * (q[i] + hper[row]) * gscale[0] / N;
}

}


namespace {

using torch::Tensor;

inline hipStream_t cur_stream() {
  return at::cuda::getCurrentCUDAStream().stream();
}

inline int64_t elementwise_blocks(int64_t work, int threads) {
  return std::max<int64_t>(1, (work + threads - 1) / threads);
}

inline int64_t reduce_blocks(int64_t work_per_group, int threads, int vec,
                             int64_t n_groups) {
  const int64_t want = (work_per_group + (int64_t)threads * vec - 1) /
                       ((int64_t)threads * vec);
  const int64_t cap = std::max<int64_t>(1, 4096 / std::max<int64_t>(n_groups, 1));
  return std::min<int64_t>(std::max<int64_t>(want, 1), cap);
}

#define DISPATCH_FT(TENSOR, NAME, ...)                                         \
  [&] {                                                                        \
    switch ((TENSOR).scalar_type()) {                                          \
      case at::ScalarType::Float: {                                            \
        using scalar_t = float;                                                \
        return __VA_ARGS__();                                                  \
      }                                                                        \
      case at::ScalarType::BFloat16: {                                         \
        using scalar_t = c10::BFloat16;                                        \
        return __VA_ARGS__();                                                  \
      }                                                                        \
      default:                                                                 \
        TORCH_CHECK(false, NAME, ": unsupported dtype ", (TENSOR).scalar_type()); \
    }                                                                          \
  }()

template <typename T>
inline T* opt_ptr(const Tensor& t, bool present) {
  return present ? t.data_ptr<T>() : nullptr;
}
template <typename T>
inline T* opt_ptr(const c10::optional<Tensor>& t) {
  return t.has_value() ? t->data_ptr<T>() : nullptr;
}


void whiten_stats_final(Tensor acc, Tensor mean, Tensor cov, int64_t g,
                        int64_t n_groups, int64_t count) {
  const int fin_threads = std::min<int64_t>(g * g, 1024);
  hipLaunchKernelGGL(dwt::whiten_stats_final_kernel, dim3(n_groups),
                     dim3(fin_threads), 0, cur_stream(), acc.data_ptr<float>(),
                     mean.data_ptr<float>(), cov.data_ptr<float>(),
                     (int)n_groups, (int)g, 1.0f / (float)count);
}

void bn_stats_final(Tensor acc, Tensor mean, Tensor istd, Tensor var_unb,
                    int64_t C, int64_t parts, int64_t count, double eps) {
  const float unb = count > 1 ? (float)count / (float)(count - 1) : 1.f;
  const int total = parts * C;
  hipLaunchKernelGGL(dwt::bn_stats_final_kernel, dim3((total + 255) / 256),
                     dim3(256), 0, cur_stream(), acc.data_ptr<float>(),
                     mean.data_ptr<float>(), istd.data_ptr<float>(),
                     var_unb.data_ptr<float>(), total, (int)C,
                     1.0f / (float)count, unb, (float)eps);
}

struct NchwParts {
  const char* name;
  int64_t parts, HW, M, numel;
  int B, C;

  NchwParts(const char* name_, const Tensor& x, int64_t parts_,
            std::initializer_list<Tensor> streamed = {})
      : name(name_), parts(parts_) {
    TORCH_CHECK(x.is_contiguous() && (x.dim() == 4 || x.dim() == 2), name,
                ": x must be contiguous (N, C, H, W) or (N, C)");
    TORCH_CHECK(parts > 0 && x.size(0) % parts == 0, name, ": batch ",
                x.size(0), " does not split into ", parts, " branches");
    for (const Tensor& t : streamed)
      TORCH_CHECK(t.scalar_type() == x.scalar_type() &&
                      t.numel() == x.numel() && t.is_contiguous(),
                  name, ": dtype, size or layout mismatch with x");
    B = x.size(0) / parts;
    C = x.size(1);
    HW = x.dim() == 4 ? x.size(2) * x.size(3) : 1;
    M = (int64_t)B * HW;
    numel = M * C;
  }
  int groups(int64_t g) const {
    TORCH_CHECK(g > 0 && C % g == 0, name, ": group size ", g,
                " does not divide C = ", C);
    return C / g;
  }
  void stacked(std::initializer_list<std::pair<Tensor, int64_t>> ops) const {
    for (const auto& [t, per] : ops)
      TORCH_CHECK(t.numel() == parts * per, name, ": a stacked operand has ",
                  t.numel(), " elements, expected ", parts * per);
  }
};

template <typename T>
struct NchwBranch {
  const NchwParts& d;
  int64_t p;
  T* operator()(const Tensor& t) const { return t.data_ptr<T>() + p * d.numel; }
  float* operator()(const Tensor& t, int64_t per) const {
    return t.data_ptr<float>() + p * per;
  }
};

template <typename T>
bool can_vectorize(const T* p, int64_t HW) {
  return HW % dwt::VecTraits<T>::W == 0 &&
         reinterpret_cast<uintptr_t>(p) % 16 == 0;
}

template <typename F>
inline void vec_launch(bool vec, F&& f) {
  if (vec) f(std::true_type{});
  else f(std::false_type{});
}

template <typename F, typename Gen>
inline void whiten_nchw_launch(const char* name, int64_t g, bool vec, F&& f,
                               Gen&& gen) {
  auto blocked = [&](auto gconst) {
    vec_launch(vec, [&](auto vconst) { f(gconst, vconst); });
  };
  switch (g) {
    case 2: blocked(std::integral_constant<int, 2>{}); break;
    case 4: blocked(std::integral_constant<int, 4>{}); break;
    case 8: blocked(std::integral_constant<int, 8>{}); break;
    default:
      TORCH_CHECK(g <= 32, name, ": unsupported group size ", g);
      gen();
  }
}

inline dim3 nchw_reduce_grid(int64_t M, int per_block, int vw, int rows) {
  return dim3(reduce_blocks(M, per_block, vw, rows), rows);
}
inline dim3 nchw_elem_grid(int64_t HW, int vw, int B, int rows) {
  return dim3((HW + (int64_t)256 * vw - 1) / ((int64_t)256 * vw), B, rows);
}

void whiten_stats_partial(Tensor x, Tensor acc, int64_t g, int64_t parts) {
  const NchwParts d("whiten_stats", x, parts);
  const int n_groups = d.groups(g);
  const int64_t n_acc = n_groups * (g + g * g);
  d.stacked({{acc, n_acc}});
  DISPATCH_FT(x, "whiten_stats", [&] {
    constexpr int VW = dwt::VecTraits<scalar_t>::W;
    for (int64_t p = 0; p < parts; ++p) {
      const NchwBranch<scalar_t> at{d, p};
      const bool vec = g <= 4 && can_vectorize(at(x), d.HW) && d.M % VW == 0;
      whiten_nchw_launch(d.name, g, vec, [&](auto gconst, auto vconst) {
        constexpr int G = decltype(gconst)::value;
        constexpr bool V = decltype(vconst)::value;
        hipLaunchKernelGGL((dwt::whiten_stats_partial_kernel<scalar_t, G, V>),
                           nchw_reduce_grid(d.M, 256, V ? VW : 1, n_groups),
                           dim3(256), 0, cur_stream(), at(x), at(acc, n_acc),
                           d.B, d.C, d.HW, d.M);
      }, [&] {
        hipLaunchKernelGGL((dwt::whiten_stats_gen_kernel<scalar_t>),
                           nchw_reduce_grid(d.M, 64, 1, n_groups), dim3(256), 0,
                           cur_stream(), at(x), at(acc, n_acc), (int)g, d.C,
                           d.HW, d.M);
      });
    }
  });
}

void whiten_apply(Tensor x, Tensor mean, Tensor W, Tensor gamma, Tensor beta,
                  Tensor out, int64_t g, bool relu, bool has_affine,
                  int64_t parts) {
  const NchwParts d("whiten_apply", x, parts, {out});
  const int n_groups = d.groups(g);
  const int64_t n_w = n_groups * g * g;
  d.stacked({{mean, d.C}, {W, n_w}});
  DISPATCH_FT(x, "whiten_apply", [&] {
    constexpr int VW = dwt::VecTraits<scalar_t>::W;
    const scalar_t* gp = opt_ptr<scalar_t>(gamma, has_affine);
    const scalar_t* bp = opt_ptr<scalar_t>(beta, has_affine);
    for (int64_t p = 0; p < parts; ++p) {
      const NchwBranch<scalar_t> at{d, p};
      const bool vec = can_vectorize(at(x), d.HW) && can_vectorize(at(out), d.HW);
      auto launch = [&](auto kernel, dim3 grid, auto... dims) {
        hipLaunchKernelGGL(kernel, grid, dim3(256), 0, cur_stream(), at(x),
                           at(mean, d.C), at(W, n_w), gp, bp, at(out), dims...,
                           relu ? 1 : 0, has_affine ? 1 : 0);
      };
      whiten_nchw_launch(d.name, g, vec, [&](auto gconst, auto vconst) {
        constexpr int G = decltype(gconst)::value;
        constexpr bool V = decltype(vconst)::value;
        launch(dwt::whiten_apply_kernel<scalar_t, G, V>,
               nchw_elem_grid(d.HW, V ? VW : 1, d.B, n_groups), d.C, d.HW);
      }, [&] {
        launch(dwt::whiten_apply_gen_kernel<scalar_t>,
               nchw_reduce_grid(d.M, 64, 1, n_groups), (int)g, d.C, d.HW, d.M);
      });
    }
  });
}

void whiten_bwd_reduce(Tensor x, Tensor dout, Tensor out, Tensor mean, Tensor W,
                       Tensor gamma, Tensor dWacc, Tensor dgb, int64_t g,
                       bool relu, bool has_affine, int64_t parts) {
  const NchwParts d("whiten_bwd_reduce", x, parts, {dout, out});
  const int n_groups = d.groups(g);
  const int64_t n_w = n_groups * g * g;
  d.stacked({{mean, d.C}, {W, n_w}, {dWacc, n_w}, {dgb, 2 * d.C}});
  DISPATCH_FT(x, "whiten_bwd_reduce", [&] {
    constexpr int VW = dwt::VecTraits<scalar_t>::W;
    const scalar_t* gp = opt_ptr<scalar_t>(gamma, has_affine);
    for (int64_t p = 0; p < parts; ++p) {
      const NchwBranch<scalar_t> at{d, p};
      const bool vec = g <= 4 && can_vectorize(at(x), d.HW) &&
// ... 352 lines not shown
            has_affine ? 1 : 0);
      });
    });
  });
}

void whiten_join_bwd_reduce_cl(Tensor x, Tensor y, Tensor ga,
                               c10::optional<Tensor> gb, Tensor mean, Tensor W,
                               Tensor gamma, Tensor gid, Tensor dWacc,
                               Tensor dgb, int64_t g, int64_t C, int64_t M,
                               bool has_affine, int64_t parts) {
  check_join_args("whiten_join_bwd_reduce_cl", x, y, ga, gb, gid,
                  parts * M * C);
  DISPATCH_FT(x, "whiten_join_bwd_reduce_cl", [&] {
    DWT_SWITCH_G(g, {
      const bool wide = whiten_wide(
          g, C, {raw_ptr(x), raw_ptr(y), raw_ptr(ga), raw_ptr(gb), raw_ptr(gid)});
      whiten_launch<scalar_t, G, kWhitenJoinReduceWide>(wide, [&](auto w) {
        constexpr bool WIDE = decltype(w)::value;
        hipLaunchKernelGGL(
            (dwt::whiten_bwd_reduce_nhwc_kernel<scalar_t, G, WIDE, true>),
            whiten_grid(kReduce, G, C, M, parts, WIDE), dim3(256), 0,
            cur_stream(), x.data_ptr<scalar_t>(), ga.data_ptr<scalar_t>(),
            y.data_ptr<scalar_t>(), opt_ptr<scalar_t>(gb),
            gid.data_ptr<scalar_t>(), mean.data_ptr<float>(),
            W.data_ptr<float>(), opt_ptr<scalar_t>(gamma, has_affine),
            (const scalar_t*)nullptr, dWacc.data_ptr<float>(),
            dgb.data_ptr<float>(), (int)C, M, 0, has_affine ? 1 : 0);
      });
    });
  });
}

void whiten_bwd_apply_cl(Tensor x, Tensor dout, Tensor mean,
                         Tensor W, Tensor gamma, Tensor beta,
                         Tensor S, Tensor corr,
                         Tensor dx, int64_t g, int64_t C, int64_t M, bool relu,
                         bool has_affine, bool train_stats, int64_t parts) {
  DISPATCH_FT(x, "whiten_bwd_apply_cl", [&] {
    DWT_SWITCH_G(g, {
      const bool wide =
          whiten_wide(g, C, {raw_ptr(x), raw_ptr(dout), raw_ptr(dx)});
      whiten_launch<scalar_t, G, kWhitenBwdApplyWide>(wide, [&](auto w) {
        constexpr bool WIDE = decltype(w)::value;
        hipLaunchKernelGGL(
            (dwt::whiten_bwd_apply_nhwc_kernel<scalar_t, G, WIDE>),
            whiten_grid(kElem, G, C, M, parts, WIDE), dim3(256), 0,
            cur_stream(), x.data_ptr<scalar_t>(), dout.data_ptr<scalar_t>(),
            mean.data_ptr<float>(), W.data_ptr<float>(),
            opt_ptr<scalar_t>(gamma, has_affine),
            opt_ptr<scalar_t>(beta, has_affine), S.data_ptr<float>(),
            corr.data_ptr<float>(), dx.data_ptr<scalar_t>(), (int)C, M,
            relu ? 1 : 0, has_affine ? 1 : 0, train_stats ? 1 : 0);
      });
    });
  });
}

void bn_stats_partial_cl(Tensor x, Tensor acc, int64_t C, int64_t M,
                         int64_t parts) {
  DISPATCH_FT(x, "bn_stats_cl", [&] {
    bn_launch<scalar_t, kBnStatsRows, kBnStatsWide>(bn_wide(C, {raw_ptr(x)}), [&](auto vc, auto rows) {
      constexpr int VC = decltype(vc)::value, R = decltype(rows)::value;
      hipLaunchKernelGGL((dwt::bn_stats_nhwc_kernel<scalar_t, VC, R>),
                         bn_grid(kReduce, C, M, parts, VC, R), dim3(256), 0,
                         cur_stream(), x.data_ptr<scalar_t>(),
                         acc.data_ptr<float>(), (int)C, M);
    });
  });
}

void bn_apply_res_cl(Tensor x, Tensor mean, Tensor istd, Tensor gamma,
                     Tensor beta, c10::optional<Tensor> res, Tensor out,
                     int64_t C, int64_t M, bool relu, bool has_affine,
                     int64_t parts) {
  TORCH_CHECK(!res.has_value() || (res->scalar_type() == x.scalar_type() &&
                                   res->numel() == x.numel()),
              "bn_apply_res_cl: res mismatch");
  DISPATCH_FT(x, "bn_apply_cl", [&] {
    const bool wide = bn_wide(C, {raw_ptr(x), raw_ptr(res), raw_ptr(out)});
    auto launch = [&](auto with_res, auto wide_rows) {
      constexpr bool RES = decltype(with_res)::value;
      constexpr bool kInUse = RES ? kBnApplyResWide : kBnApplyWide;
      bn_launch<scalar_t, decltype(wide_rows)::value, kInUse>(wide, [&](auto vc, auto rows) {
        constexpr int VC = decltype(vc)::value, R = decltype(rows)::value;
        hipLaunchKernelGGL((dwt::bn_apply_nhwc_kernel<scalar_t, VC, R, RES>),
                           bn_grid(kElem, C, M, parts, VC, R), dim3(256), 0,
                           cur_stream(), x.data_ptr<scalar_t>(),
                           opt_ptr<scalar_t>(res), mean.data_ptr<float>(),
                           istd.data_ptr<float>(),
                           opt_ptr<scalar_t>(gamma, has_affine),
                           opt_ptr<scalar_t>(beta, has_affine),
                           out.data_ptr<scalar_t>(), (int)C, M, relu ? 1 : 0,
                           has_affine ? 1 : 0);
      });
    };
    if (res.has_value())
      launch(std::true_type{}, std::integral_constant<int, kBnApplyResRows>{});
    else
      launch(std::false_type{}, std::integral_constant<int, kBnApplyRows>{});
  });
}

void bn_apply_cl(Tensor x, Tensor mean, Tensor istd, Tensor gamma, Tensor beta,
                 Tensor out, int64_t C, int64_t M, bool relu, bool has_affine,
                 int64_t parts) {
  bn_apply_res_cl(x, mean, istd, gamma, beta, c10::nullopt, out, C, M, relu,
                  has_affine, parts);
}

void bn_bwd_reduce_cl(Tensor x, Tensor dout, Tensor mean,
                      Tensor istd, Tensor gamma, Tensor beta,
                      Tensor sums, int64_t C, int64_t M,
                      bool relu, bool has_affine, int64_t parts) {
  DISPATCH_FT(x, "bn_bwd_reduce_cl", [&] {
    const bool wide = bn_wide(C, {raw_ptr(x), raw_ptr(dout)});
    bn_launch<scalar_t, kBnReduceRows, kBnReduceWide>(wide, [&](auto vc, auto rows) {
      constexpr int VC = decltype(vc)::value, R = decltype(rows)::value;
      hipLaunchKernelGGL(
          (dwt::bn_bwd_reduce_nhwc_kernel<scalar_t, VC, R, false>),
          bn_grid(kReduce, C, M, parts, VC, R), dim3(256), 0, cur_stream(),
          x.data_ptr<scalar_t>(), dout.data_ptr<scalar_t>(),
          (const scalar_t*)nullptr, (const scalar_t*)nullptr,
          (scalar_t*)nullptr, mean.data_ptr<float>(), istd.data_ptr<float>(),
          opt_ptr<scalar_t>(gamma, has_affine),
          opt_ptr<scalar_t>(beta, has_affine), sums.data_ptr<float>(), (int)C,
          M, relu ? 1 : 0, has_affine ? 1 : 0);
    });
  });
}

void bn_join_bwd_reduce_cl(Tensor x, Tensor y, Tensor ga,
                           c10::optional<Tensor> gb, Tensor mean, Tensor istd,
                           Tensor gid, Tensor sums, int64_t C, int64_t M,
                           int64_t parts) {
  check_join_args("bn_join_bwd_reduce_cl", x, y, ga, gb, gid, parts * M * C);
  DISPATCH_FT(x, "bn_join_bwd_reduce_cl", [&] {
    const bool wide = bn_wide(
        C, {raw_ptr(x), raw_ptr(y), raw_ptr(ga), raw_ptr(gb), raw_ptr(gid)});
    bn_launch<scalar_t, kBnReduceRows, kBnJoinReduceWide>(wide, [&](auto vc, auto rows) {
      constexpr int VC = decltype(vc)::value, R = decltype(rows)::value;
      hipLaunchKernelGGL(
          (dwt::bn_bwd_reduce_nhwc_kernel<scalar_t, VC, R, true>),
          bn_grid(kReduce, C, M, parts, VC, R), dim3(256), 0, cur_stream(),
          x.data_ptr<scalar_t>(), ga.data_ptr<scalar_t>(),
          y.data_ptr<scalar_t>(), opt_ptr<scalar_t>(gb),
          gid.data_ptr<scalar_t>(), mean.data_ptr<float>(),
          istd.data_ptr<float>(), (const scalar_t*)nullptr,
          (const scalar_t*)nullptr, sums.data_ptr<float>(), (int)C, M, 0, 0);
    });
  });
}

void bn_bwd_apply_cl(Tensor x, Tensor dout, Tensor mean,
                     Tensor istd, Tensor gamma, Tensor beta,
                     Tensor sums, Tensor dx,
                     int64_t C, int64_t M, bool relu, bool has_affine,
                     bool use_batch, int64_t parts, int64_t count) {
  DISPATCH_FT(x, "bn_bwd_apply_cl", [&] {
    const bool wide = bn_wide(C, {raw_ptr(x), raw_ptr(dout), raw_ptr(dx)});
    bn_launch<scalar_t, kBnBwdApplyRows, kBnBwdApplyWide>(wide, [&](auto vc, auto rows) {
      constexpr int VC = decltype(vc)::value, R = decltype(rows)::value;
      hipLaunchKernelGGL((dwt::bn_bwd_apply_nhwc_kernel<scalar_t, VC, R>),
                         bn_grid(kElem, C, M, parts, VC, R), dim3(256), 0,
                         cur_stream(), x.data_ptr<scalar_t>(),
                         dout.data_ptr<scalar_t>(), mean.data_ptr<float>(),
                         istd.data_ptr<float>(),
                         opt_ptr<scalar_t>(gamma, has_affine),
                         opt_ptr<scalar_t>(beta, has_affine),
                         sums.data_ptr<float>(), dx.data_ptr<scalar_t>(),
                         (int)C, M, 1.0f / (float)count, relu ? 1 : 0,
                         has_affine ? 1 : 0, use_batch ? 1 : 0);
    });
  });
}

void matfn_chol_fwd(Tensor cov, Tensor W, Tensor L, double eps) {
  const int n_groups = cov.size(0);
  const int g = cov.size(1);
  TORCH_CHECK(g <= MATFN_MAX_G, "group size too large for matfn");
  hipLaunchKernelGGL(dwt::matfn_chol_fwd_kernel, dim3(n_groups), dim3(64), 0,
                     cur_stream(), cov.data_ptr<float>(), W.data_ptr<float>(),
                     L.data_ptr<float>(), g, (float)eps);
}

void matfn_chol_bwd(Tensor dW, Tensor W, Tensor L, Tensor gdb, Tensor S,
                    Tensor corr, double eps, double inv_m) {
  const int n_groups = W.size(0);
  const int g = W.size(1);
  hipLaunchKernelGGL(dwt::matfn_chol_bwd_kernel, dim3(n_groups), dim3(64), 0,
                     cur_stream(), dW.data_ptr<float>(), W.data_ptr<float>(),
                     L.data_ptr<float>(), gdb.data_ptr<float>(),
                     S.data_ptr<float>(), corr.data_ptr<float>(), g, (float)eps,
                     (float)inv_m);
}

void matfn_ns_fwd(Tensor cov, Tensor W, Tensor ys, Tensor zs, Tensor svals,
                  double eps, int64_t iters) {
  const int n_groups = cov.size(0);
  const int g = cov.size(1);
  TORCH_CHECK(g <= MATFN_MAX_G, "group size too large for matfn");
  hipLaunchKernelGGL(dwt::matfn_ns_fwd_kernel, dim3(n_groups), dim3(64), 0,
                     cur_stream(), cov.data_ptr<float>(), W.data_ptr<float>(),
                     ys.data_ptr<float>(), zs.data_ptr<float>(),
                     svals.data_ptr<float>(), g, (float)eps, (int)iters);
}

void matfn_ns_bwd(Tensor dW, Tensor W, Tensor ys, Tensor zs, Tensor svals,
                  Tensor gdb, Tensor S, Tensor corr, double eps, double inv_m,
                  int64_t iters) {
  const int n_groups = W.size(0);
  const int g = W.size(1);
  hipLaunchKernelGGL(dwt::matfn_ns_bwd_kernel, dim3(n_groups), dim3(64), 0,
                     cur_stream(), dW.data_ptr<float>(), W.data_ptr<float>(),
                     ys.data_ptr<float>(), zs.data_ptr<float>(),
                     svals.data_ptr<float>(), gdb.data_ptr<float>(),
                     S.data_ptr<float>(), corr.data_ptr<float>(), g, (float)eps,
                     (float)inv_m, (int)iters);
}

void maxpool_cl_fwd(Tensor x, Tensor out, Tensor idx, int64_t C, int64_t H,
                    int64_t W, int64_t P, int64_t Q, int64_t KS,
                    int64_t stride, int64_t pad) {
  const int64_t total = out.numel();
  DISPATCH_FT(x, "maxpool_cl_fwd", [&] {
    constexpr int VC = dwt::VecTraits<scalar_t>::W;
    if (C % VC == 0) {
      const int64_t chunks = total / VC;
      hipLaunchKernelGGL((dwt::maxpool_nhwc_fwd_vec_kernel<scalar_t, VC>),
                         dim3(elementwise_blocks(chunks, 256)), dim3(256), 0,
                         cur_stream(), x.data_ptr<scalar_t>(),
                         out.data_ptr<scalar_t>(), idx.data_ptr<uint8_t>(),
                         (int)C, (int)H, (int)W, (int)P, (int)Q, (int)KS,
                         (int)stride, (int)pad, chunks);
    } else {
      hipLaunchKernelGGL((dwt::maxpool_nhwc_fwd_kernel<scalar_t>),
                         dim3(elementwise_blocks(total, 256)), dim3(256), 0,
                         cur_stream(), x.data_ptr<scalar_t>(),
                         out.data_ptr<scalar_t>(), idx.data_ptr<uint8_t>(),
                         (int)C, (int)H, (int)W, (int)P, (int)Q, (int)KS,
                         (int)stride, (int)pad, total);
    }
  });
}

void maxpool_cl_bwd(Tensor dout, Tensor idx, Tensor dx, int64_t C, int64_t H,
                    int64_t W, int64_t P, int64_t Q, int64_t KS,
                    int64_t stride, int64_t pad) {
  const int64_t total_in = dx.numel();
  DISPATCH_FT(dout, "maxpool_cl_bwd", [&] {
    constexpr int VC = dwt::VecTraits<scalar_t>::W;
    if (C % VC == 0) {
      const int64_t chunks = total_in / VC;
      hipLaunchKernelGGL((dwt::maxpool_nhwc_bwd_vec_kernel<scalar_t, VC>),
                         dim3(elementwise_blocks(chunks, 256)), dim3(256), 0,
                         cur_stream(), dout.data_ptr<scalar_t>(),
                         idx.data_ptr<uint8_t>(), dx.data_ptr<scalar_t>(),
                         (int)C, (int)H, (int)W, (int)P, (int)Q, (int)KS,
                         (int)stride, (int)pad, chunks);
    } else {
      hipLaunchKernelGGL((dwt::maxpool_nhwc_bwd_kernel<scalar_t>),
                         dim3(elementwise_blocks(total_in, 256)), dim3(256), 0,
                         cur_stream(), dout.data_ptr<scalar_t>(),
                         idx.data_ptr<uint8_t>(), dx.data_ptr<scalar_t>(),
                         (int)C, (int)H, (int)W, (int)P, (int)Q, (int)KS,
                         (int)stride, (int)pad, total_in);
    }
  });
}

void gap_cl_fwd(Tensor x, Tensor out, int64_t C, int64_t HW, int64_t N) {
  DISPATCH_FT(x, "gap_cl_fwd", [&] {
    dim3 grid((C + 63) / 64, N);
    hipLaunchKernelGGL((dwt::gap_nhwc_fwd_kernel<scalar_t>), grid, dim3(64), 0,
                       cur_stream(), x.data_ptr<scalar_t>(),
                       out.data_ptr<scalar_t>(), (int)C, HW, (int)N);
  });
}

void gap_cl_bwd(Tensor dout, Tensor dx, int64_t C, int64_t HW) {
  const int64_t total = dx.numel();
  DISPATCH_FT(dout, "gap_cl_bwd", [&] {
    hipLaunchKernelGGL((dwt::gap_nhwc_bwd_kernel<scalar_t>),
                       dim3(elementwise_blocks(total, 256)), dim3(256), 0,
                       cur_stream(), dout.data_ptr<scalar_t>(),
                       dx.data_ptr<scalar_t>(), (int)C, HW, total);
  });
}

void add_relu_fwd(Tensor a, Tensor b, Tensor out) {
  const int64_t n = a.numel();
  DISPATCH_FT(a, "add_relu_fwd", [&] {
    constexpr int VW = dwt::VecTraits<scalar_t>::W;
    const bool vec = (n % VW == 0) &&
        (reinterpret_cast<uintptr_t>(a.data_ptr()) % 16 == 0) &&
        (reinterpret_cast<uintptr_t>(b.data_ptr()) % 16 == 0);
    const int64_t per = vec ? (n + 256 * VW - 1) / (256 * VW)
                            : (n + 255) / 256;
    if (vec)
      hipLaunchKernelGGL((dwt::add_relu_fwd_kernel<scalar_t, true>), dim3(per),
                         dim3(256), 0, cur_stream(), a.data_ptr<scalar_t>(),
                         b.data_ptr<scalar_t>(), out.data_ptr<scalar_t>(), n);
    else
      hipLaunchKernelGGL((dwt::add_relu_fwd_kernel<scalar_t, false>), dim3(per),
                         dim3(256), 0, cur_stream(), a.data_ptr<scalar_t>(),
                         b.data_ptr<scalar_t>(), out.data_ptr<scalar_t>(), n);
  });
}

void add_relu_bwd(Tensor dout, Tensor out, Tensor din) {
  const int64_t n = dout.numel();
  DISPATCH_FT(dout, "add_relu_bwd", [&] {
    constexpr int VW = dwt::VecTraits<scalar_t>::W;
    const bool vec = (n % VW == 0) &&
        (reinterpret_cast<uintptr_t>(dout.data_ptr()) % 16 == 0);
    const int64_t per = vec ? (n + 256 * VW - 1) / (256 * VW)
                            : (n + 255) / 256;
    if (vec)
      hipLaunchKernelGGL((dwt::add_relu_bwd_kernel<scalar_t, true>), dim3(per),
                         dim3(256), 0, cur_stream(), dout.data_ptr<scalar_t>(),
                         out.data_ptr<scalar_t>(), din.data_ptr<scalar_t>(), n);
    else
      hipLaunchKernelGGL((dwt::add_relu_bwd_kernel<scalar_t, false>), dim3(per),
                         dim3(256), 0, cur_stream(), dout.data_ptr<scalar_t>(),
                         out.data_ptr<scalar_t>(), din.data_ptr<scalar_t>(), n);
  });
}

void fused_sgd(Tensor desc, int64_t n_chunks, double lr, double momentum,
               double wd, bool bf16_params, bool master, bool zero_grad,
               bool first_step) {
  auto lp = [&](auto tconst, auto mconst) {
    using T = typename decltype(tconst)::type;
    constexpr bool M = decltype(mconst)::value;
    hipLaunchKernelGGL((dwt::sgd_kernel<T, M>), dim3(n_chunks), dim3(256), 0,
                       cur_stream(), desc.data_ptr<int64_t>(), (float)lr,
                       (float)momentum, (float)wd, zero_grad ? 1 : 0,
                       first_step ? 1 : 0);
  };
  struct FT { using type = float; };
  struct BT { using type = c10::BFloat16; };
  if (bf16_params) {
    if (master) lp(BT{}, std::true_type{}); else lp(BT{}, std::false_type{});
  } else {
    if (master) lp(FT{}, std::true_type{}); else lp(FT{}, std::false_type{});
  }
}

void fused_adam(Tensor desc, int64_t n_chunks, double lr, double beta1,
                double beta2, double eps, double wd, double bc1, double bc2,
                bool bf16_params, bool master, bool zero_grad) {
  auto lp = [&](auto tconst, auto mconst) {
    using T = typename decltype(tconst)::type;
    constexpr bool M = decltype(mconst)::value;
    hipLaunchKernelGGL((dwt::adam_kernel<T, M>), dim3(n_chunks), dim3(256), 0,
                       cur_stream(), desc.data_ptr<int64_t>(), (float)lr,
                       (float)beta1, (float)beta2, (float)eps, (float)wd,
                       (float)bc1, (float)bc2, zero_grad ? 1 : 0);
  };
  struct FT { using type = float; };
  struct BT { using type = c10::BFloat16; };
  if (bf16_params) {
    if (master) lp(BT{}, std::true_type{}); else lp(BT{}, std::false_type{});
  } else {
    if (master) lp(FT{}, std::true_type{}); else lp(FT{}, std::false_type{});
  }
}

void ema_update(Tensor rm, Tensor a, Tensor rv, Tensor b, double momentum) {
  const int64_t n1 = rm.numel(), n2 = rv.numel();
  hipLaunchKernelGGL(dwt::ema_update_kernel,
                     dim3(elementwise_blocks(n1 + n2, 256)), dim3(256), 0,
                     cur_stream(), rm.data_ptr<float>(), a.data_ptr<float>(),
                     n1, rv.data_ptr<float>(), b.data_ptr<float>(), n2,
                     (float)momentum);
}


void mec_fwd(Tensor x, Tensor y, Tensor lx, Tensor ly, Tensor amin, Tensor loss) {
  const int N = x.size(0), K = x.size(1);
  const int rows_per_block = 4;
  hipLaunchKernelGGL(dwt::mec_fwd_kernel,
                     dim3((N + rows_per_block - 1) / rows_per_block),
                     dim3(rows_per_block * 64), 0, cur_stream(),
                     x.data_ptr<float>(), y.data_ptr<float>(),
                     lx.data_ptr<float>(), ly.data_ptr<float>(),
                     amin.data_ptr<int>(), loss.data_ptr<float>(), N, K);
}

void mec_bwd(Tensor lx, Tensor ly, Tensor amin, Tensor gscale, Tensor dx, Tensor dy) {
  const int N = lx.size(0), K = lx.size(1);
  const int64_t total = (int64_t)N * K;
  hipLaunchKernelGGL(dwt::mec_bwd_kernel, dim3(elementwise_blocks(total, 256)),
                     dim3(256), 0, cur_stream(), lx.data_ptr<float>(),
                     ly.data_ptr<float>(), amin.data_ptr<int>(),
                     gscale.data_ptr<float>(), dx.data_ptr<float>(),
                     dy.data_ptr<float>(), N, K);
}

void entropy_fwd(Tensor x, Tensor q, Tensor hper, Tensor loss) {
  const int N = x.size(0), K = x.size(1);
  const int rows_per_block = 4;
  hipLaunchKernelGGL(dwt::entropy_fwd_kernel,
                     dim3((N + rows_per_block - 1) / rows_per_block),
                     dim3(rows_per_block * 64), 0, cur_stream(),
                     x.data_ptr<float>(), q.data_ptr<float>(),
                     hper.data_ptr<float>(), loss.data_ptr<float>(), N, K);
}

void ce_fwd(Tensor x, Tensor target, Tensor q, Tensor loss) {
  const int N = x.size(0), K = x.size(1);
  const int rows_per_block = 4;
  hipLaunchKernelGGL(dwt::ce_fwd_kernel,
                     dim3((N + rows_per_block - 1) / rows_per_block),
                     dim3(rows_per_block * 64), 0, cur_stream(),
                     x.data_ptr<float>(), target.data_ptr<int64_t>(),
                     q.data_ptr<float>(), loss.data_ptr<float>(), N, K);
}

void ce_bwd(Tensor q, Tensor target, Tensor gscale, Tensor dx) {
  const int N = q.size(0), K = q.size(1);
  hipLaunchKernelGGL(dwt::ce_bwd_kernel,
                     dim3(elementwise_blocks((int64_t)N * K, 256)), dim3(256),
                     0, cur_stream(), q.data_ptr<float>(),
                     target.data_ptr<int64_t>(), gscale.data_ptr<float>(),
                     dx.data_ptr<float>(), N, K);
}

void entropy_bwd(Tensor q, Tensor hper, Tensor gscale, Tensor dx) {
  const int N = q.size(0), K = q.size(1);
  const int64_t total = (int64_t)N * K;
  hipLaunchKernelGGL(dwt::entropy_bwd_kernel,
                     dim3(elementwise_blocks(total, 256)), dim3(256), 0,
                     cur_stream(), q.data_ptr<float>(), hper.data_ptr<float>(),
                     gscale.data_ptr<float>(), dx.data_ptr<float>(), N, K);
}

}

void mfma_gemm(torch::Tensor a, torch::Tensor bt, torch::Tensor bias,
               torch::Tensor out, bool relu, bool has_bias);
void mfma_conv2d_fwd(torch::Tensor x, torch::Tensor wgt, torch::Tensor bias,
                     torch::Tensor out, int64_t N, int64_t H, int64_t W,
                     int64_t Cin, int64_t P, int64_t Q, int64_t Cout,
                     int64_t KH, int64_t KW, int64_t stride, int64_t pad,
                     bool relu, bool has_bias);
void mfma_conv2d_fwd_fused(torch::Tensor x, torch::Tensor wgt,
                           torch::Tensor bias, torch::Tensor res,
                           torch::Tensor out, int64_t N, int64_t H, int64_t W,
                           int64_t Cin, int64_t P, int64_t Q, int64_t Cout,
                           int64_t KH, int64_t KW, int64_t stride, int64_t pad,
                           bool relu, bool has_res);
void conv1x1_stats(torch::Tensor x, torch::Tensor wgt, torch::Tensor out,
                   torch::Tensor acc, int64_t kind, int64_t g, int64_t parts,
                   int64_t max_workgroups);
void mfma_conv2d_dgrad(torch::Tensor dy, torch::Tensor wd, torch::Tensor dx,
                       int64_t N, int64_t H, int64_t W, int64_t Cin,
                       int64_t P, int64_t Q, int64_t Cdy, int64_t KH,
                       int64_t KW, int64_t stride, int64_t pad);
void mfma_conv2d_wgrad(torch::Tensor dy, torch::Tensor x, torch::Tensor dw,
                       torch::Tensor ws, int64_t N, int64_t H, int64_t W,
                       int64_t Cin, int64_t P, int64_t Q, int64_t Cout,
                       int64_t KH, int64_t KW, int64_t stride, int64_t pad);
void set_dense_glds(bool on);
bool dense_glds_selected();
int64_t dense_glds_launches();

void assemble_views(torch::Tensor images, torch::Tensor src_index,
                    torch::Tensor top, torch::Tensor left, torch::Tensor flags,
                    torch::Tensor inv_affine, torch::Tensor out,
                    std::vector<double> mean, std::vector<double> std_);

PYBIND11_MODULE(TORCH_EXTENSION_NAME, m) {
  m.def("assemble_views", &assemble_views);
  m.def("mfma_gemm", &mfma_gemm);
  m.def("mfma_conv2d_fwd", &mfma_conv2d_fwd);
  m.def("mfma_conv2d_fwd_fused", &mfma_conv2d_fwd_fused);
  m.def("conv1x1_stats", &conv1x1_stats);
  m.def("mfma_conv2d_dgrad", &mfma_conv2d_dgrad);
  m.def("mfma_conv2d_wgrad", &mfma_conv2d_wgrad);
  m.def("set_dense_glds", &set_dense_glds);
  m.def("dense_glds_selected", &dense_glds_selected);
  m.def("dense_glds_launches", &dense_glds_launches);
  m.def("whiten_stats_partial", &whiten_stats_partial);
  m.def("whiten_stats_partial_cl", &whiten_stats_partial_cl);
  m.def("whiten_stats_final", &whiten_stats_final);
  m.def("bn_stats_partial", &bn_stats_partial);
  m.def("bn_stats_partial_cl", &bn_stats_partial_cl);
  m.def("bn_stats_final", &bn_stats_final);
  m.def("whiten_apply_cl", &whiten_apply_cl);
  m.def("whiten_bwd_reduce_cl", &whiten_bwd_reduce_cl);
  m.def("whiten_bwd_apply_cl", &whiten_bwd_apply_cl);
  m.def("bn_apply_cl", &bn_apply_cl);
  m.def("bn_bwd_reduce_cl", &bn_bwd_reduce_cl);
  m.def("bn_bwd_apply_cl", &bn_bwd_apply_cl);
  m.def("whiten_apply_res_cl", &whiten_apply_res_cl);
  m.def("bn_apply_res_cl", &bn_apply_res_cl);
  m.def("whiten_join_bwd_reduce_cl", &whiten_join_bwd_reduce_cl);
  m.def("bn_join_bwd_reduce_cl", &bn_join_bwd_reduce_cl);
  m.def("set_norm_wide", &set_norm_wide);
  m.def("norm_wide_selected", &norm_wide_selected);
  m.def("matfn_chol_fwd", &matfn_chol_fwd);
  m.def("matfn_chol_bwd", &matfn_chol_bwd);
  m.def("matfn_ns_fwd", &matfn_ns_fwd);
  m.def("matfn_ns_bwd", &matfn_ns_bwd);
  m.def("whiten_apply", &whiten_apply);
  m.def("whiten_bwd_reduce", &whiten_bwd_reduce);
  m.def("whiten_bwd_apply", &whiten_bwd_apply);
  m.def("bn_apply", &bn_apply);
  m.def("bn_bwd_reduce", &bn_bwd_reduce);
  m.def("bn_bwd_apply", &bn_bwd_apply);
  m.def("ema_update", &ema_update);
  m.def("maxpool_cl_fwd", &maxpool_cl_fwd);
  m.def("maxpool_cl_bwd", &maxpool_cl_bwd);
  m.def("gap_cl_fwd", &gap_cl_fwd);
  m.def("gap_cl_bwd", &gap_cl_bwd);
  m.def("add_relu_fwd", &add_relu_fwd);
  m.def("add_relu_bwd", &add_relu_bwd);
  m.def("fused_sgd", &fused_sgd);
  m.def("fused_adam", &fused_adam);
  m.def("mec_fwd", &mec_fwd);
  m.def("mec_bwd", &mec_bwd);
  m.def("entropy_fwd", &entropy_fwd);
  m.def("ce_fwd", &ce_fwd);
  m.def("ce_bwd", &ce_bwd);
  m.def("entropy_bwd", &entropy_bwd);
}
```

### dwt_amd/models/sites.py

```python
from __future__ import annotations

from typing import Optional, Sequence

import torch
import torch.nn as nn

from ..ops import functional as Fdwt
from ..ops.whitening import WhiteningScaleShift, WTransform2d
from ..ops.batch_norm import _DomainBatchNorm


def _wh_of(mod: nn.Module) -> WTransform2d:
    return mod.wh if isinstance(mod, WhiteningScaleShift) else mod


def norm_site(
    x: torch.Tensor,
    branches: Sequence[nn.Module],
    gamma: Optional[torch.Tensor],
    beta: Optional[torch.Tensor],
    training: bool,
    relu: bool,
    eval_branch: int = 1,
    residual: Optional[torch.Tensor] = None,
    stats_acc: Optional[torch.Tensor] = None,
):
    if residual is not None:
        assert relu, "a residual join applies its ReLU after the add"
    if not training:
        stats_acc = None
    first = branches[0]
    if training:
        use = list(branches)
        parts = len(use)
    else:
        use = [branches[min(eval_branch, len(branches) - 1)]]
        parts = 1

    if isinstance(first, (WhiteningScaleShift, WTransform2d)):
        whs = [_wh_of(b) for b in use]
        w0 = whs[0]
        kw = dict(parts=parts, num_groups=w0.num_groups, eps=w0.eps,
                  momentum=w0.momentum, training=training, mode=w0.mode,
                  track_running_stats=w0.track_running_stats,
                  stats_acc=stats_acc)
        rms = [w.running_mean for w in whs]
        rvs = [w.running_variance for w in whs]
        if residual is not None:
            return Fdwt.norm_join("whiten", x, residual, gamma, beta, rms, rvs,
                                  **kw)
        return Fdwt.whiten_multi(x, gamma, beta, rms, rvs, relu=relu, **kw)

    if isinstance(first, (_DomainBatchNorm, nn.modules.batchnorm._BatchNorm)):
        momentum = first.momentum if first.momentum is not None else 0.0
        if training and first.track_running_stats:
            for b in use:
                if b.num_batches_tracked is not None:
                    b.num_batches_tracked += 1
            if first.momentum is None:
                momentum = 1.0 / first.num_batches_tracked.item()
        spatial = x.dim() == 4
        gshape = (-1, 1, 1) if spatial else (1, -1)
        gamma = gamma.reshape(gshape) if gamma is not None else None
        beta = beta.reshape(gshape) if beta is not None else None
        rms = [b.running_mean for b in use] if first.track_running_stats else None
        rvs = [b.running_var for b in use] if first.track_running_stats else None
        kw = dict(parts=parts, eps=first.eps, momentum=momentum,
                  training=training,
                  track_running_stats=first.track_running_stats,
                  stats_acc=stats_acc)
        if residual is not None:
            return Fdwt.norm_join("bn", x, residual, gamma, beta, rms, rvs, **kw)
        return Fdwt.batch_norm_multi(x, gamma, beta, rms, rvs, relu=relu, **kw)

    raise TypeError(f"unsupported norm branch type {type(first)}")
```

### dwt_amd/ops/batch_norm.py

```python
from __future__ import annotations

import torch
import torch.nn as nn
import torch.nn.init as init
from torch.nn.parameter import Parameter

from . import functional as Fdwt


class _DomainBatchNorm(nn.Module):
    def __init__(self, num_features, running_m=None, running_v=None, eps=1e-5,
                 momentum=0.1, affine=True, track_running_stats=True):
        super().__init__()
        self.num_features = num_features
        self.eps = eps
        self.momentum = momentum
        self.affine = affine
        self.track_running_stats = track_running_stats
        if affine:
            self.weight = Parameter(torch.Tensor(num_features))
            self.bias = Parameter(torch.Tensor(num_features))
        else:
            self.register_parameter("weight", None)
            self.register_parameter("bias", None)
        if track_running_stats:
            self.register_buffer("running_mean",
                                 running_m if running_m is not None else torch.zeros(num_features))
            self.register_buffer("running_var",
                                 running_v if running_v is not None else torch.ones(num_features))
            self.register_buffer("num_batches_tracked", torch.tensor(0, dtype=torch.long))
        else:
            self.register_parameter("running_mean", None)
            self.register_parameter("running_var", None)
            self.register_parameter("num_batches_tracked", None)
        self.reset_parameters()

    def _apply(self, fn, recurse=True):
        super()._apply(fn, recurse)
        for name in ("running_mean", "running_var"):
            b = self._buffers.get(name)
            if b is not None and b.is_floating_point() and b.dtype != torch.float32:
                self._buffers[name] = b.float()
        return self

    def reset_running_stats(self):
        if self.track_running_stats:
            self.num_batches_tracked.zero_()

    def reset_parameters(self):
        self.reset_running_stats()
        if self.affine:
            init.uniform_(self.weight)
            init.zeros_(self.bias)

    def _check_input_dim(self, x):
        raise NotImplementedError

    def forward(self, x):
        self._check_input_dim(x)
        return self._bn(x)

    def _bn(self, x):
        momentum = self.momentum if self.momentum is not None else 0.0
        if self.training and self.track_running_stats:
            self.num_batches_tracked += 1
            if self.momentum is None:
                momentum = 1.0 / self.num_batches_tracked.item()

        squeeze = False
        if x.dim() == 2:
            x4 = x
        elif x.dim() == 3:
            x4 = x.unsqueeze(-1)
            squeeze = True
        else:
            x4 = x
        gamma = self.weight.reshape(-1, *([1] * (x4.dim() - 2))) if self.affine else None
        beta = self.bias.reshape(-1, *([1] * (x4.dim() - 2))) if self.affine else None
        out = Fdwt.batch_norm_multi(
            x4, gamma, beta,
            [self.running_mean] if self.track_running_stats else None,
            [self.running_var] if self.track_running_stats else None,
            parts=1, eps=self.eps, momentum=momentum, training=self.training,
            relu=False, track_running_stats=self.track_running_stats)
        return out.squeeze(-1) if squeeze else out


class DomainBatchNorm1d(_DomainBatchNorm):
    def _check_input_dim(self, x):
        if x.dim() != 2 and x.dim() != 3:
            raise ValueError(f"expected 2D or 3D input (got {x.dim()}D input)")


class DomainBatchNorm2d(_DomainBatchNorm):
    def _check_input_dim(self, x):
        if x.dim() != 4:
            raise ValueError(f"expected 4D input (got {x.dim()}D input)")


class DomainBatchNorm3d(_DomainBatchNorm):
    def _check_input_dim(self, x):
        if x.dim() != 5:
            raise ValueError(f"expected 5D input (got {x.dim()}D input)")

    def forward(self, x):
        self._check_input_dim(x)
        n, c, d, h, w = x.shape
        out = self._bn(x.reshape(n, c, d * h, w))
        return out.reshape(n, c, d, h, w)


BatchNorm1d = DomainBatchNorm1d
BatchNorm2d = DomainBatchNorm2d
BatchNorm3d = DomainBatchNorm3d
```

### dwt_amd/ops/functional.py

```python
from __future__ import annotations

import os
from typing import List, Optional, Sequence

import torch
import torch.nn.functional as F

from . import oracle




def matfn_chol_forward(cov_s: torch.Tensor):
    ell = torch.linalg.cholesky(cov_s)
    eye = torch.eye(ell.shape[-1], dtype=ell.dtype, device=ell.device).expand_as(ell)
    w = torch.linalg.solve_triangular(ell, eye, upper=False)
    return w, ell


def matfn_chol_backward(w: torch.Tensor, ell: torch.Tensor, w_bar: torch.Tensor):
    l_bar = torch.tril(-w.transpose(-1, -2) @ w_bar @ w.transpose(-1, -2))
    s = ell.transpose(-1, -2) @ l_bar
    phi = torch.tril(s)
    phi = phi - 0.5 * torch.diag_embed(phi.diagonal(dim1=-2, dim2=-1))
# ... 263 lines not shown
            return dispatch.whiten_multi(x, gamma, beta, running_means,
                                         running_vars, cfg, stats_acc)
        dispatch.require_or_warn("whiten_multi")
    return WhitenMulti.apply(x, gamma, beta, running_means, running_vars, cfg)




class BatchNormMulti(torch.autograd.Function):

    @staticmethod
    def forward(ctx, x, gamma, beta, running_means, running_vars, cfg):
        parts = cfg["parts"]
        eps = cfg["eps"]
        momentum = cfg["momentum"]
        training = cfg["training"]
        relu = cfg["relu"]
        track = cfg.get("track_running_stats", True)
        use_batch = training or not track

        spatial = x.dim() == 4
        n = x.shape[0]
        c = x.shape[1]
        b = n // parts
        comp_dtype = torch.float32 if x.dtype != torch.float64 else torch.float64

        xhat = torch.empty_like(x)
        means, invstds = [], []
        red_dims = (0, 2, 3) if spatial else (0,)
        stats_sync = cfg.get("stats_sync", False) and use_batch
        dist, world = _dist_world() if stats_sync else (None, 1)
        ctx.world = world
        for p in range(parts):
            sl = slice(p * b, (p + 1) * b)
            xp = x[sl].to(comp_dtype)
            if use_batch:
                if dist is not None:
                    pack = torch.stack([xp.sum(dim=red_dims),
                                        (xp * xp).sum(dim=red_dims)])
                    dist.all_reduce(pack)
                    cnt = (xp.numel() // c) * world
                    m = pack[0] / cnt
                    var = (pack[1] / cnt - m * m).clamp_min(0)
                else:
                    m = xp.mean(dim=red_dims)
                    var = xp.var(dim=red_dims, unbiased=False)
                    cnt = xp.numel() // c
                if training and track and running_means is not None:
                    with torch.no_grad():
                        rm, rv = running_means[p], running_vars[p]
                        var_unb = var * (cnt / max(cnt - 1, 1))
                        rm.mul_(1 - momentum).add_(m.to(rm.dtype), alpha=momentum)
                        rv.mul_(1 - momentum).add_(var_unb.to(rv.dtype), alpha=momentum)
            else:
                m = running_means[p].to(comp_dtype)
                var = running_vars[p].to(comp_dtype)
            istd = torch.rsqrt(var + eps)
            shape = (1, c, 1, 1) if spatial else (1, c)
            xhat[sl] = ((xp - m.reshape(shape)) * istd.reshape(shape)).to(x.dtype)
            means.append(m)
            invstds.append(istd)

        if gamma is not None:
            out = xhat * gamma.to(x.dtype) + beta.to(x.dtype)
        else:
            out = xhat
        if relu:
            out = torch.relu(out)

        ctx.cfg = cfg
        ctx.means = means
        ctx.invstds = invstds
        ctx.spatial = spatial
        ctx.has_affine = gamma is not None
        ctx.comp_dtype = comp_dtype
        ctx.save_for_backward(x, gamma, xhat, out)
        return out

    @staticmethod
    def backward(ctx, dout):
        cfg = ctx.cfg
        parts, relu, training = cfg["parts"], cfg["relu"], cfg["training"]
        track = cfg.get("track_running_stats", True)
        use_batch = training or not track
        x, gamma, xhat, out = ctx.saved_tensors
        comp_dtype = ctx.comp_dtype
        spatial = ctx.spatial
        n, c = x.shape[0], x.shape[1]
        b = n // parts
        red_dims = (0, 2, 3) if spatial else (0,)
        shape = (1, c, 1, 1) if spatial else (1, c)

        dy = dout * (out > 0).to(dout.dtype) if relu else dout
        if ctx.has_affine:
            dgamma = (dy * xhat).sum(dim=red_dims).reshape(gamma.shape).to(gamma.dtype)
            dbeta = dy.sum(dim=red_dims).reshape(gamma.shape).to(gamma.dtype)
            dxhat_all = (dy * gamma.to(dy.dtype)).to(comp_dtype)
        else:
            dgamma = dbeta = None
            dxhat_all = dy.to(comp_dtype)

        dx = torch.empty_like(x)
        for p in range(parts):
            sl = slice(p * b, (p + 1) * b)
            dxh = dxhat_all[sl]
            istd = ctx.invstds[p].reshape(shape)
            xh = xhat[sl].to(comp_dtype)
            if use_batch:
                mean_dxh = dxh.mean(dim=red_dims, keepdim=True)
                mean_dxh_xh = (dxh * xh).mean(dim=red_dims, keepdim=True)
                world = getattr(ctx, "world", 1)
                if cfg.get("stats_sync", False) and world > 1:
                    import torch.distributed as dist
                    pack = torch.stack([mean_dxh, mean_dxh_xh])
                    dist.all_reduce(pack)
                    mean_dxh, mean_dxh_xh = pack[0] / world, pack[1] / world
                dxp = (dxh - mean_dxh - xh * mean_dxh_xh) * istd
            else:
                dxp = dxh * istd
            dx[sl] = dxp.to(x.dtype)
        return dx, dgamma, dbeta, None, None, None


def _bn_cfg(
    *,
    parts: int,
    eps: float = 1e-5,
    momentum: float = 0.1,
    training: bool = True,
    relu: bool = False,
    track_running_stats: bool = True,
) -> dict:
    cfg = dict(parts=parts, eps=eps, momentum=momentum, training=training,
               relu=relu, track_running_stats=track_running_stats)
    if os.environ.get("DWT_AMD_STATS_SYNC") == "1":
        cfg["stats_sync"] = True
    return cfg


def batch_norm_multi(
    x: torch.Tensor,
    gamma: Optional[torch.Tensor],
    beta: Optional[torch.Tensor],
    running_means: Optional[Sequence[torch.Tensor]],
    running_vars: Optional[Sequence[torch.Tensor]],
    *,
    parts: int,
    eps: float = 1e-5,
    momentum: float = 0.1,
    training: bool = True,
    relu: bool = False,
    track_running_stats: bool = True,
    stats_acc: Optional[torch.Tensor] = None,
) -> torch.Tensor:
    cfg = _bn_cfg(parts=parts, eps=eps, momentum=momentum, training=training,
                  relu=relu, track_running_stats=track_running_stats)
    if x.is_cuda:
        from ..kernels import dispatch
        if dispatch.available():
            return dispatch.batch_norm_multi(x, gamma, beta, running_means,
                                             running_vars, cfg, stats_acc)
        dispatch.require_or_warn("batch_norm_multi")
    return BatchNormMulti.apply(x, gamma, beta, running_means, running_vars, cfg)




class MecLossFn(torch.autograd.Function):

    @staticmethod
    def forward(ctx, x, y):
        ct = torch.float64 if x.dtype == torch.float64 else torch.float32
        lx = F.log_softmax(x.to(ct), dim=1)
        ly = F.log_softmax(y.to(ct), dim=1)
        per = -0.5 * (lx + ly)
        vals, idx = per.min(dim=1)
        ctx.save_for_backward(lx, ly, idx)
        ctx.dtypes = (x.dtype, y.dtype)
        return vals.mean()

    @staticmethod
    def backward(ctx, dloss):
        lx, ly, idx = ctx.saved_tensors
        n, k = lx.shape
        onehot = F.one_hot(idx, k).to(lx.dtype)
        dx = (lx.exp() - onehot) * (dloss.to(lx.dtype) / (2 * n))
        dy = (ly.exp() - onehot) * (dloss.to(ly.dtype) / (2 * n))
        return dx.to(ctx.dtypes[0]), dy.to(ctx.dtypes[1])


class EntropyLossFn(torch.autograd.Function):

    @staticmethod
    def forward(ctx, x):
        ct = torch.float64 if x.dtype == torch.float64 else torch.float32
        q = F.log_softmax(x.to(ct), dim=1)
        p = q.exp()
        h_per = -(p * q).sum(dim=1)
        ctx.save_for_backward(p, q, h_per)
        ctx.dtype = x.dtype
        return h_per.mean()

    @staticmethod
    def backward(ctx, dloss):
        p, q, h_per = ctx.saved_tensors
        n = p.shape[0]
        dx = -p * (q + h_per.unsqueeze(1)) * (dloss.to(p.dtype) / n)
        return dx.to(ctx.dtype)


def mec_loss(x: torch.Tensor, y: torch.Tensor) -> torch.Tensor:
    if x.is_cuda:
        from ..kernels import dispatch
        if dispatch.available():
            return dispatch.mec_loss(x, y)
        dispatch.require_or_warn("mec_loss")
    return MecLossFn.apply(x, y)


def entropy_loss(x: torch.Tensor) -> torch.Tensor:
    if x.is_cuda:
        from ..kernels import dispatch
        if dispatch.available():
            return dispatch.entropy_loss(x)
        dispatch.require_or_warn("entropy_loss")
    return EntropyLossFn.apply(x)




class AddReluFn(torch.autograd.Function):

    @staticmethod
    def _mf(t):
        if t.dim() == 4 and t.is_contiguous(memory_format=torch.channels_last) \
                and not t.is_contiguous():
            return torch.channels_last
        return torch.contiguous_format

    @staticmethod
    def forward(ctx, a, b):
        if a.is_cuda and a.dtype in (torch.float32, torch.bfloat16):
            from ..kernels import dispatch
            if dispatch.available():
                ext = dispatch.ext()
                mf = AddReluFn._mf(a)
                ac = a.contiguous(memory_format=mf) if a.dim() == 4 else a.contiguous()
                bc = b.contiguous(memory_format=mf) if b.dim() == 4 else b.contiguous()
                out = torch.empty_like(ac)
                ext.add_relu_fwd(ac, bc, out)
                ctx.save_for_backward(out)
                ctx.use_hip = True
                return out
        out = torch.relu(a + b)
        ctx.save_for_backward(out)
        ctx.use_hip = False
        return out

    @staticmethod
    def backward(ctx, dout):
        (out,) = ctx.saved_tensors
        if ctx.use_hip:
            from ..kernels import dispatch
            ext = dispatch.ext()
            mf = AddReluFn._mf(out)
            dout = dout.contiguous(memory_format=mf) if dout.dim() == 4 \
                else dout.contiguous()
            din = torch.empty_like(out)
            ext.add_relu_bwd(dout, out, din)
            return din, din
        mask = (out > 0).to(dout.dtype)
        d = dout * mask
        return d, d


def add_relu(a: torch.Tensor, b: torch.Tensor) -> torch.Tensor:
    return AddReluFn.apply(a, b)


def fused_join_enabled() -> bool:
    return os.environ.get("DWT_AMD_FUSED_JOIN", "1") != "0"


def norm_join(
    kind: str,
    x: torch.Tensor,
    identity: torch.Tensor,
    gamma: Optional[torch.Tensor],
    beta: Optional[torch.Tensor],
    running_means: Optional[Sequence[torch.Tensor]],
    running_vars: Optional[Sequence[torch.Tensor]],
    **kw,
):
    assert kind in ("whiten", "bn"), kind
    kw = dict(kw, relu=False)
    stats_acc = kw.pop("stats_acc", None)
    if x.is_cuda and fused_join_enabled():
        from ..kernels import dispatch
        if dispatch.available():
            from ..kernels import hip_ops
            cfg = _whiten_cfg(**kw) if kind == "whiten" else _bn_cfg(**kw)
            if hip_ops.join_supported(kind, x, identity, cfg):
                fn = hip_ops.whiten_join if kind == "whiten" \
                    else hip_ops.batch_norm_join
                return fn(x, identity, gamma, beta, running_means,
                          running_vars, cfg, stats_acc)
    multi = whiten_multi if kind == "whiten" else batch_norm_multi
    y = add_relu(multi(x, gamma, beta, running_means, running_vars,
                       stats_acc=stats_acc, **kw),
                 identity)
    return y, y


def ce_loss(logits: torch.Tensor, target: torch.Tensor) -> torch.Tensor:
    if logits.is_cuda:
        from ..kernels import dispatch
        if dispatch.available():
            return dispatch.ce_loss(logits, target)
        dispatch.require_or_warn("ce_loss")
    return F.nll_loss(F.log_softmax(logits.float(), dim=1), target)
```

Before: 9622 images/sec.

## Fold running-stat EMA, batch counters and affine grads into norm kernels

Folds the running-mean/var EMA update and the num_batches_tracked increment into the stats-finalization kernels for whitening and BN. The per-domain affine gradient reductions (dgamma/dbeta) move into the matrix-function backward and BN backward-apply kernels, replacing separate small torch ops and launches per norm site. This cuts kernel launches and host overhead in a model with many norm layers. It adds new overloaded bindings, and the extra branching and pointer tables add complexity.

```diff
diff --git a/dwt_amd/kernels/dispatch.py b/dwt_amd/kernels/dispatch.py
--- a/dwt_amd/kernels/dispatch.py
+++ b/dwt_amd/kernels/dispatch.py
@@ -69,10 +69,10 @@
 
 
 def batch_norm_multi(x, gamma, beta, running_means, running_vars, cfg,
-                     stats_acc=None):
+                     stats_acc=None, counters=None):
     from . import hip_ops
     return hip_ops.batch_norm_multi(x, gamma, beta, running_means,
-                                    running_vars, cfg, stats_acc)
+                                    running_vars, cfg, stats_acc, counters)
 
 
 def mec_loss(x, y):
diff --git a/dwt_amd/kernels/hip_ops.py b/dwt_amd/kernels/hip_ops.py
--- a/dwt_amd/kernels/hip_ops.py
+++ b/dwt_amd/kernels/hip_ops.py
@@ -4,7 +4,7 @@
 import torch
 
 from . import dispatch
-from ..ops.functional import _dist_world
+from ..ops.functional import _dist_world, site_fold_enabled
 
 _GEN_G_MAX = 32
 _warned = set()
@@ -60,6 +60,41 @@
             new_var.reshape(rv.shape).to(rv.dtype), alpha=momentum)
 
 
+_FOLD_MAX_PARTS = 8
+
+
+def _ema_foldable(x, rms, rvs, parts, training, track, momentum):
+    if not (training and track) or rms is None or rvs is None \
+            or momentum is None or not site_fold_enabled():
+        return False
+    if x.dtype not in (torch.float32, torch.bfloat16) \
+            or not 1 <= parts <= _FOLD_MAX_PARTS \
+            or len(rms) < parts or len(rvs) < parts:
+        return False
+    return all(t is not None and t.dtype == torch.float32
+               and t.is_contiguous() and t.device == x.device
+               for t in (*rms[:parts], *rvs[:parts]))
+
+
+def bn_fold_takes_counters(x, rms, rvs, counters, parts, training, track,
+                           momentum):
+    if counters is None or len(counters) != parts:
+        return False
+    if not all(k is not None and k.dtype == torch.int64 and k.dim() == 0
+               and k.device == x.device for k in counters):
+        return False
+    return _ema_foldable(x, rms, rvs, parts, training, track, momentum)
+
+
+def _advance(counters, cfg):
+    if counters is not None and cfg["training"] \
+            and cfg.get("track_running_stats", True):
+        with torch.no_grad():
+            for k in counters:
+                if k is not None:
+                    k += 1
+
+
 def _warn_once(key, msg):
     if key not in _warned:
         _warned.add(key)
@@ -93,7 +128,7 @@
 
     @staticmethod
     def forward(ctx, x, gamma, beta, running_means, running_vars, cfg,
-                stats_acc=None, res=None):
+                stats_acc=None, counters=None, res=None):
         ext = _ext()
         parts = cfg["parts"]
         g = x.shape[1] // cfg["num_groups"]
@@ -121,6 +156,7 @@
         ctx_count = m_count * world
 
         out = torch.empty_like(x)
+        fold_ema = False
         if use_batch:
             acc = _usable_stats_acc(stats_acc, x, layout, training,
                                     ng_all * (g + g * g))
@@ -134,7 +170,15 @@
                 _allreduce(acc)
             mean = torch.empty(parts * c, device=dev, dtype=torch.float32)
             cov = torch.empty(ng_all, g, g, device=dev, dtype=torch.float32)
-            ext.whiten_stats_final(acc, mean, cov, g, ng_all, ctx_count)
+            fold_ema = _ema_foldable(x, running_means, running_vars, parts,
+                                     training, track, momentum)
+            if fold_ema:
+                ext.whiten_stats_final_ema(acc, mean, cov,
+                                           list(running_means[:parts]),
+                                           list(running_vars[:parts]), g,
+                                           ng_all, parts, ctx_count, momentum)
+            else:
+                ext.whiten_stats_final(acc, mean, cov, g, ng_all, ctx_count)
         else:
             mean = torch.stack([_f32c(running_means[p]).reshape(c)
                                 for p in range(parts)]).reshape(-1).contiguous()
@@ -164,7 +208,7 @@
             ext.whiten_apply(x, mean, wmat, gflat, bflat, out, g, relu,
                              has_affine, parts)
 
-        if training and track and running_means is not None:
+        if training and track and running_means is not None and not fold_ema:
             with torch.no_grad():
                 for p in range(parts):
                     _ema_update(ext, running_means[p], mean[p * c:(p + 1) * c],
@@ -189,7 +233,7 @@
     @staticmethod
     def backward(ctx, dout):
         dx, _, dgamma, dbeta = _HipWhitenMulti.run_backward(ctx, dout)
-        return dx, dgamma, dbeta, None, None, None, None
+        return dx, dgamma, dbeta, None, None, None, None, None
 
     @staticmethod
     def run_backward(ctx, dout, gb=None, join=False):
@@ -237,24 +281,34 @@
                                   dgb.reshape(-1), g, relu, ctx.has_affine,
                                   parts)
 
+        fold = use_batch and ctx.sync_world == 1 and site_fold_enabled()
+        dgamma = dbeta = None
         if use_batch:
-            gdb = (ctx.gflat.float().unsqueeze(0) * dgb[:, 1]) if ctx.has_affine \
-                else dgb[:, 1]
-            gdb = gdb.reshape(-1).contiguous()
-            dW_in = dW
-            if ctx.sync_world > 1:
-                dW_in = _allreduce(dW.clone())
-                gdb = _allreduce(gdb.clone())
             S = torch.empty(ng_all, g, g, device=dev, dtype=torch.float32)
             corr = torch.empty(parts * c, device=dev, dtype=torch.float32)
             inv_m = 1.0 / m_count
-            if mode == "chol":
-                ext.matfn_chol_bwd(dW_in, wmat, ctx.saved_mat, gdb, S, corr,
-                                   eps, inv_m)
+            saved = (ctx.saved_mat,) if mode == "chol" else ctx.saved_mat
+            tail = (eps, inv_m) if mode == "chol" else (eps, inv_m, ns_iters)
+            matfn_bwd = ext.matfn_chol_bwd if mode == "chol" \
+                else ext.matfn_ns_bwd
+            if fold:
+                aff = (ctx.gflat,) * 3
+                if ctx.has_affine:
+                    dgamma = torch.empty(gamma.shape, device=dev,
+                                         dtype=gamma.dtype)
+                    dbeta = torch.empty_like(dgamma)
+                    aff = (ctx.gflat, dgamma, dbeta)
+                matfn_bwd(dW, wmat, *saved, dgb, *aff, S, corr, *tail,
+                          ctx.has_affine, parts)
             else:
-                ys, zs, svals = ctx.saved_mat
-                ext.matfn_ns_bwd(dW_in, wmat, ys, zs, svals, gdb, S, corr,
-                                 eps, inv_m, ns_iters)
+                gdb = (ctx.gflat.float().unsqueeze(0) * dgb[:, 1]) \
+                    if ctx.has_affine else dgb[:, 1]
+                gdb = gdb.reshape(-1).contiguous()
+                dW_in = dW
+                if ctx.sync_world > 1:
+                    dW_in = _allreduce(dW.clone())
+                    gdb = _allreduce(gdb.clone())
+                matfn_bwd(dW_in, wmat, *saved, gdb, S, corr, *tail)
         else:
             S = torch.empty(0, device=dev)
             corr = torch.empty(0, device=dev)
@@ -267,11 +321,9 @@
             ext.whiten_bwd_apply(x, dout, out, mean, wmat, ctx.gflat, S, corr,
                                  dx, g, relu, ctx.has_affine, use_batch, parts)
 
-        if ctx.has_affine:
+        if ctx.has_affine and not fold:
             dgamma = dgb[:, 0].sum(0).reshape(gamma.shape).to(gamma.dtype)
             dbeta = dgb[:, 1].sum(0).reshape(gamma.shape).to(gamma.dtype)
-        else:
-            dgamma = dbeta = None
         return dx, gid, dgamma, dbeta
 
 
@@ -289,15 +341,15 @@
 
 
 def whiten_join(x, identity, gamma, beta, running_means, running_vars, cfg,
-                stats_acc=None):
+                stats_acc=None, counters=None):
     return _HipWhitenJoin.apply(x, identity, gamma, beta, running_means,
-                                running_vars, cfg, stats_acc)
+                                running_vars, cfg, stats_acc, counters)
 
 
 def batch_norm_join(x, identity, gamma, beta, running_means, running_vars, cfg,
-                    stats_acc=None):
+                    stats_acc=None, counters=None):
     return _HipBatchNormJoin.apply(x, identity, gamma, beta, running_means,
-                                   running_vars, cfg, stats_acc)
+                                   running_vars, cfg, stats_acc, counters)
 
 
 def whiten_multi(x, gamma, beta, running_means, running_vars, cfg,
@@ -316,7 +368,7 @@
 class _HipBatchNormMulti(torch.autograd.Function):
     @staticmethod
     def forward(ctx, x, gamma, beta, running_means, running_vars, cfg,
-                stats_acc=None, res=None):
+                stats_acc=None, counters=None, res=None):
         ext = _ext()
         parts = cfg["parts"]
         eps, momentum = cfg["eps"], cfg["momentum"]
@@ -354,9 +406,21 @@
             mean = torch.empty(parts * c, device=dev, dtype=torch.float32)
             istd = torch.empty(parts * c, device=dev, dtype=torch.float32)
             var_unb = torch.empty(parts * c, device=dev, dtype=torch.float32)
-            ext.bn_stats_final(acc, mean, istd, var_unb, c, parts, cnt_total,
-                               eps)
-            if training and track and running_means is not None:
+            fold_ema = bn_fold_takes_counters(x, running_means, running_vars,
+                                              counters, parts, training, track,
+                                              momentum)
+            if fold_ema:
+                ext.bn_stats_final_ema(acc, mean, istd, var_unb,
+                                       list(running_means[:parts]),
+                                       list(running_vars[:parts]),
+                                       list(counters), c, parts, cnt_total,
+                                       eps, momentum)
+                counters = None
+            else:
+                ext.bn_stats_final(acc, mean, istd, var_unb, c, parts,
+                                   cnt_total, eps)
+            if training and track and running_means is not None \
+                    and not fold_ema:
                 with torch.no_grad():
                     for p in range(parts):
                         _ema_update(ext, running_means[p],
@@ -368,6 +432,7 @@
             var = torch.stack([_f32c(running_vars[p]).reshape(c)
                                for p in range(parts)]).reshape(-1)
             istd = torch.rsqrt(var + eps).contiguous()
+        _advance(counters, cfg)
 
         if res is not None:
             assert layout == "cl" and x.dim() == 4
@@ -398,7 +463,7 @@
     @staticmethod
     def backward(ctx, dout):
         dx, _, dgamma, dbeta = _HipBatchNormMulti.run_backward(ctx, dout)
-        return dx, dgamma, dbeta, None, None, None, None
+        return dx, dgamma, dbeta, None, None, None, None, None
 
     @staticmethod
     def run_backward(ctx, dout, gb=None, join=False):
@@ -437,6 +502,17 @@
         apply_sums = sums.reshape(-1)
         if ctx.sync_world > 1:
             apply_sums = _allreduce(apply_sums.clone())
+        fold = layout == "cl" and ctx.has_affine and site_fold_enabled() \
+            and gamma.dtype == x.dtype
+        if fold:
+            dgamma = torch.empty(gamma.shape, device=dev, dtype=gamma.dtype)
+            dbeta = torch.empty(gamma.shape, device=dev, dtype=gamma.dtype)
+            ext.bn_bwd_apply_cl(x, dout, mean, istd, ctx.gflat, ctx.bflat,
+                                apply_sums, dx, dgamma, dbeta,
+                                sums.reshape(-1), c, ctx.cnt, relu,
+                                ctx.has_affine, ctx.use_batch, parts,
+                                ctx.cnt_total)
+            return dx, gid, dgamma, dbeta
         if layout == "cl":
             ext.bn_bwd_apply_cl(x, dout, mean, istd, ctx.gflat, ctx.bflat,
                                 apply_sums, dx, c, ctx.cnt, relu,
@@ -458,20 +534,20 @@
 def _join_function(name, site):
 
     def forward(ctx, x, identity, gamma, beta, running_means, running_vars,
-                cfg, stats_acc=None):
+                cfg, stats_acc=None, counters=None):
         ctx.set_materialize_grads(False)
         res = identity.detach()
         y = site.forward(ctx, x, gamma, beta, running_means, running_vars,
-                         cfg, stats_acc, res=res)
+                         cfg, stats_acc, counters, res=res)
         return y, y.view_as(y)
 
     def backward(ctx, ga, gb):
         if ga is None and gb is None:
-            return (None,) * 8
+            return (None,) * 9
         if ga is None:
             ga, gb = gb, None
         dx, gid, dgamma, dbeta = site.run_backward(ctx, ga, gb, join=True)
-        return dx, gid, dgamma, dbeta, None, None, None, None
+        return dx, gid, dgamma, dbeta, None, None, None, None, None
 
     return type(name, (torch.autograd.Function,),
                 {"__doc__": _join_function.__doc__,
@@ -484,12 +560,13 @@
 
 
 def batch_norm_multi(x, gamma, beta, running_means, running_vars, cfg,
-                     stats_acc=None):
+                     stats_acc=None, counters=None):
     if x.dtype not in (torch.float32, torch.bfloat16):
         from ..ops.functional import BatchNormMulti
+        _advance(counters, cfg)
         return BatchNormMulti.apply(x, gamma, beta, running_means, running_vars, cfg)
     return _HipBatchNormMulti.apply(x, gamma, beta, running_means, running_vars,
-                                    cfg, stats_acc)
+                                    cfg, stats_acc, counters)
 
 
 class _HipMecLoss(torch.autograd.Function):
diff --git a/dwt_amd/kernels/src/dwt_kernels.hip b/dwt_amd/kernels/src/dwt_kernels.hip
--- a/dwt_amd/kernels/src/dwt_kernels.hip
+++ b/dwt_amd/kernels/src/dwt_kernels.hip
@@ -29,6 +29,22 @@
   unsigned int rounded = u.i + 0x7fffu + lsb;
   *reinterpret_cast<unsigned short*>(p) = static_cast<unsigned short>(rounded >> 16);
 }
+
+DEV_INLINE float ema_step(float r, float v, float momentum) {
+#pragma clang fp contract(off)
+  return (1.f - momentum) * r + momentum * v;
+}
+
+DEV_INLINE float sub_prod(float a, float b, float c) {
+  return __builtin_fmaf(-b, c, a);
+}
+
+constexpr int kFoldMaxParts = 8;
+struct FoldPtrs {
+  float* rm[kFoldMaxParts];
+  float* rv[kFoldMaxParts];
+  int64_t* cnt[kFoldMaxParts];
+};
 
 template <typename T> struct VecTraits;
 template <> struct VecTraits<float> {
@@ -162,8 +178,36 @@
   const float mi = gacc[i] * inv_m;
   const float mj = gacc[j] * inv_m;
   const float pij = (j <= i) ? gacc[g + i * g + j] : gacc[g + j * g + i];
-  cov[((int64_t)grp * g + i) * g + j] = pij * inv_m - mi * mj;
+  cov[((int64_t)grp * g + i) * g + j] = sub_prod(pij * inv_m, mi, mj);
   if (j == 0) mean[grp * g + i] = mi;
+}
+
+__global__ void whiten_stats_final_ema_kernel(
+    const float* __restrict__ acc, float* __restrict__ mean,
+    float* __restrict__ cov, int ngp, int g, int parts, float inv_m,
+    float momentum, FoldPtrs f) {
+  const int i = threadIdx.x / g, j = threadIdx.x % g;
+  if (i >= g) return;
+  const int64_t e = ((int64_t)blockIdx.x * g + i) * g + j;
+#pragma unroll
+  for (int p = 0; p < kFoldMaxParts; ++p) {
+    if (p >= parts) break;
+    const int64_t grp = (int64_t)p * ngp + blockIdx.x;
+    const float* gacc = acc + grp * (g + g * g);
+    const float mi = gacc[i] * inv_m;
+    const float mj = gacc[j] * inv_m;
+    const float pij = (j <= i) ? gacc[g + i * g + j] : gacc[g + j * g + i];
+    const float cv = sub_prod(pij * inv_m, mi, mj);
+    cov[(grp * g + i) * g + j] = cv;
+    float* rv = f.rv[p];
+    rv[e] = ema_step(rv[e], cv, momentum);
+    if (j == 0) {
+      mean[grp * g + i] = mi;
+      float* rm = f.rm[p];
+      const int c = blockIdx.x * g + i;
+      rm[c] = ema_step(rm[c], mi, momentum);
+    }
+  }
 }
 
 
@@ -440,9 +484,39 @@
   }
 }
 
+template <typename T>
+struct GdbOperand {
+  const float* flat;
+  const float* dgb;
+  const T* gamma;
+  T* dgamma;
+  T* dbeta;
+  int C, parts;
+  DEV_INLINE float operator()(int idx) const {
+    if (dgb == nullptr) return flat[idx];
+    const int p = idx / C, c = idx - p * C;
+    const float d = dgb[((int64_t)p * 2 + 1) * C + c];
+    return gamma != nullptr ? ldf(gamma + c) * d : d;
+  }
+  DEV_INLINE void write_affine_grads(int grp, int g) const {
+    if (dgb == nullptr || dgamma == nullptr || (int64_t)grp * g >= C) return;
+    for (int i = threadIdx.x; i < g; i += blockDim.x) {
+      const int c = grp * g + i;
+      float dg = dgb[c], db = dgb[C + c];
+      for (int p = 1; p < parts; ++p) {
+        dg += dgb[(int64_t)p * 2 * C + c];
+        db += dgb[((int64_t)p * 2 + 1) * C + c];
+      }
+      stf(dgamma + c, dg);
+      stf(dbeta + c, db);
+    }
+  }
+};
+
+template <typename T>
 __global__ void matfn_chol_bwd_kernel(
     const float* __restrict__ dW, const float* __restrict__ W,
-    const float* __restrict__ L, const float* __restrict__ gdb,
+    const float* __restrict__ L, const GdbOperand<T> gdb,
     float* __restrict__ S, float* __restrict__ corr,
     int g, float eps, float inv_m) {
   __shared__ float sW[MATFN_MAX_G * MATFN_MAX_G];
@@ -495,9 +569,10 @@
   }
   for (int i = t; i < g; i += 64) {
     float v = 0.f;
-    for (int j = 0; j < g; ++j) v += sW[j * g + i] * gdb[grp * g + j];
+    for (int j = 0; j < g; ++j) v += sW[j * g + i] * gdb(grp * g + j);
     corr[grp * g + i] = v * inv_m;
   }
+  gdb.write_affine_grads(grp, g);
 }
 
 __global__ void matfn_ns_fwd_kernel(
@@ -561,10 +636,11 @@
   for (int e = t; e < g * g; e += 64) Wout[base + e] = Z[e] * inv_sqrt_s;
 }
 
+template <typename T>
 __global__ void matfn_ns_bwd_kernel(
     const float* __restrict__ dW, const float* __restrict__ W,
     const float* __restrict__ ys, const float* __restrict__ zs,
-    const float* __restrict__ svals, const float* __restrict__ gdb,
+    const float* __restrict__ svals, const GdbOperand<T> gdb,
     float* __restrict__ S, float* __restrict__ corr,
     int g, float eps, float inv_m, int iters) {
   __shared__ float YB[MATFN_MAX_G * MATFN_MAX_G];
@@ -642,9 +718,10 @@
   }
   for (int i = t; i < g; i += 64) {
     float v = 0.f;
-    for (int j = 0; j < g; ++j) v += W[base + j * g + i] * gdb[grp * g + j];
+    for (int j = 0; j < g; ++j) v += W[base + j * g + i] * gdb(grp * g + j);
     corr[grp * g + i] = v * inv_m;
   }
+  gdb.write_affine_grads(grp, g);
 }
 
 
@@ -1529,14 +1606,30 @@
     const float* __restrict__ istd, const T* __restrict__ gamma,
     const T* __restrict__ beta,
     const float* __restrict__ sums, T* __restrict__ dx, int C, int64_t M,
-    float inv_m, int relu, int has_affine, int use_batch) {
+    float inv_m, int relu, int has_affine, int use_batch,
+    T* __restrict__ dgamma, T* __restrict__ dbeta, const float* lsums,
+    int parts) {
   const int part = blockIdx.y;
+  const BnLanes<VC> L(C);
+  if (dgamma != nullptr && blockIdx.x == 0 && part == 0 &&
+      L.row_in_block == 0) {
+#pragma unroll
+    for (int k = 0; k < VC; ++k) {
+      const int c = L.c0 + k;
+      float db = lsums[c], dg = lsums[C + c];
+      for (int p = 1; p < parts; ++p) {
+        db += lsums[(int64_t)p * 2 * C + c];
+        dg += lsums[(int64_t)p * 2 * C + C + c];
+      }
+      stf(dbeta + c, db);
+      stf(dgamma + c, dg);
+    }
+  }
   const int64_t poff = (int64_t)part * M * C;
   x += poff; dout += poff; dx += poff;
   mean += (int64_t)part * C;
   istd += (int64_t)part * C;
   sums += (int64_t)part * 2 * C;
-  const BnLanes<VC> L(C);
   float mu[VC], is[VC], gm[VC], bt[VC], mdy[VC], mdyxh[VC];
 #pragma unroll
   for (int k = 0; k < VC; ++k) {
@@ -1614,10 +1707,36 @@
   const int p = i / Cper, c = i % Cper;
   const int64_t base = (int64_t)p * 2 * Cper;
   const float mu = acc[base + c] * inv_m;
-  float var = fmaxf(acc[base + Cper + c] * inv_m - mu * mu, 0.f);
+  float var = fmaxf(sub_prod(acc[base + Cper + c] * inv_m, mu, mu), 0.f);
   mean[i] = mu;
   istd[i] = rsqrtf(var + eps);
   var_unb[i] = var * unb_scale;
+}
+
+__global__ void bn_stats_final_ema_kernel(
+    const float* __restrict__ acc, float* __restrict__ mean,
+    float* __restrict__ istd, float* __restrict__ var_unb,
+    int Cper, int parts, float inv_m, float unb_scale, float eps,
+    float momentum, FoldPtrs f) {
+  const int c = blockIdx.x * blockDim.x + threadIdx.x;
+  if (c >= Cper) return;
+#pragma unroll
+  for (int p = 0; p < kFoldMaxParts; ++p) {
+    if (p >= parts) break;
+    const int64_t base = (int64_t)p * 2 * Cper;
+    const int64_t i = (int64_t)p * Cper + c;
+    const float mu = acc[base + c] * inv_m;
+    float var = fmaxf(sub_prod(acc[base + Cper + c] * inv_m, mu, mu), 0.f);
+    mean[i] = mu;
+    istd[i] = rsqrtf(var + eps);
+    const float vu = var * unb_scale;
+    var_unb[i] = vu;
+    float* rm = f.rm[p];
+    float* rv = f.rv[p];
+    rm[c] = ema_step(rm[c], mu, momentum);
+    rv[c] = ema_step(rv[c], vu, momentum);
+    if (c == 0 && f.cnt[p] != nullptr) *f.cnt[p] += 1;
+  }
 }
 
 template <typename T, bool VECTOR>
@@ -1747,10 +1866,10 @@
                                   float momentum) {
   const int64_t i = (int64_t)blockIdx.x * blockDim.x + threadIdx.x;
   if (i < n1) {
-    rm[i] = (1.f - momentum) * rm[i] + momentum * a[i];
+    rm[i] = ema_step(rm[i], a[i], momentum);
   } else if (i < n1 + n2) {
     const int64_t j = i - n1;
-    rv[j] = (1.f - momentum) * rv[j] + momentum * b[j];
+    rv[j] = ema_step(rv[j], b[j], momentum);
   }
 }
 
@@ -2208,6 +2327,72 @@
                      mean.data_ptr<float>(), istd.data_ptr<float>(),
                      var_unb.data_ptr<float>(), total, (int)C,
                      1.0f / (float)count, unb, (float)eps);
+}
+
+dwt::FoldPtrs fold_ptrs(const char* name, const std::vector<Tensor>& rms,
+                        const std::vector<Tensor>& rvs,
+                        const std::vector<Tensor>& counters, int64_t parts,
+                        int64_t n_mean, int64_t n_var) {
+  TORCH_CHECK(parts >= 1 && parts <= dwt::kFoldMaxParts, name, ": parts ", parts);
+  TORCH_CHECK((int64_t)rms.size() == parts && (int64_t)rvs.size() == parts,
+              name, ": one running mean and var per branch");
+  TORCH_CHECK(counters.empty() || (int64_t)counters.size() == parts, name,
+              ": one counter per branch, or none");
+  dwt::FoldPtrs f = {};
+  for (int64_t p = 0; p < parts; ++p) {
+    for (const Tensor* t : {&rms[p], &rvs[p]})
+      TORCH_CHECK(t->is_cuda() && t->scalar_type() == at::ScalarType::Float &&
+                      t->is_contiguous(),
+                  name, ": running buffers must be fp32 contiguous on the GPU");
+    TORCH_CHECK(rms[p].numel() == n_mean && rvs[p].numel() == n_var, name,
+                ": running buffer size");
+    f.rm[p] = rms[p].data_ptr<float>();
+    f.rv[p] = rvs[p].data_ptr<float>();
+    if (!counters.empty()) {
+      const Tensor& k = counters[p];
+      TORCH_CHECK(k.is_cuda() && k.scalar_type() == at::ScalarType::Long &&
+                      k.numel() == 1,
+                  name, ": counters must be int64 scalars on the GPU");
+      f.cnt[p] = k.data_ptr<int64_t>();
+    }
+  }
+  return f;
+}
+
+void whiten_stats_final_ema(Tensor acc, Tensor mean, Tensor cov,
+                            std::vector<Tensor> rms, std::vector<Tensor> rvs,
+                            int64_t g, int64_t n_groups, int64_t parts,
+                            int64_t count, double momentum) {
+  TORCH_CHECK(parts >= 1 && n_groups % parts == 0, "whiten_stats_final_ema: groups");
+  const int64_t ngp = n_groups / parts;
+  TORCH_CHECK(acc.numel() == n_groups * (g + g * g) &&
+                  mean.numel() == n_groups * g && cov.numel() == n_groups * g * g,
+              "whiten_stats_final_ema: statistics size");
+  const dwt::FoldPtrs f = fold_ptrs("whiten_stats_final_ema", rms, rvs, {},
+                                    parts, ngp * g, ngp * g * g);
+  const int fin_threads = std::min<int64_t>(g * g, 1024);
+  hipLaunchKernelGGL(dwt::whiten_stats_final_ema_kernel, dim3(ngp),
+                     dim3(fin_threads), 0, cur_stream(), acc.data_ptr<float>(),
+                     mean.data_ptr<float>(), cov.data_ptr<float>(), (int)ngp,
+                     (int)g, (int)parts, 1.0f / (float)count, (float)momentum,
+                     f);
+}
+
+void bn_stats_final_ema(Tensor acc, Tensor mean, Tensor istd, Tensor var_unb,
+                        std::vector<Tensor> rms, std::vector<Tensor> rvs,
+                        std::vector<Tensor> counters, int64_t C, int64_t parts,
+                        int64_t count, double eps, double momentum) {
+  TORCH_CHECK(acc.numel() == parts * 2 * C && mean.numel() == parts * C &&
+                  istd.numel() == parts * C && var_unb.numel() == parts * C,
+              "bn_stats_final_ema: statistics size");
+  const dwt::FoldPtrs f =
+      fold_ptrs("bn_stats_final_ema", rms, rvs, counters, parts, C, C);
+  const float unb = count > 1 ? (float)count / (float)(count - 1) : 1.f;
+  hipLaunchKernelGGL(dwt::bn_stats_final_ema_kernel, dim3((C + 255) / 256),
+                     dim3(256), 0, cur_stream(), acc.data_ptr<float>(),
+                     mean.data_ptr<float>(), istd.data_ptr<float>(),
+                     var_unb.data_ptr<float>(), (int)C, (int)parts,
+                     1.0f / (float)count, unb, (float)eps, (float)momentum, f);
 }
 
 struct NchwParts {
@@ -2866,11 +3051,23 @@
   });
 }
 
-void bn_bwd_apply_cl(Tensor x, Tensor dout, Tensor mean,
-                     Tensor istd, Tensor gamma, Tensor beta,
-                     Tensor sums, Tensor dx,
-                     int64_t C, int64_t M, bool relu, bool has_affine,
-                     bool use_batch, int64_t parts, int64_t count) {
+void bn_bwd_apply_cl_impl(Tensor x, Tensor dout, Tensor mean,
+                          Tensor istd, Tensor gamma, Tensor beta,
+                          Tensor sums, Tensor dx,
+                          const std::vector<Tensor>& grads,
+                          int64_t C, int64_t M, bool relu, bool has_affine,
+                          bool use_batch, int64_t parts, int64_t count) {
+  const bool with_grads = !grads.empty();
+  if (with_grads) {
+    for (int k = 0; k < 2; ++k)
+      TORCH_CHECK(grads[k].scalar_type() == x.scalar_type() &&
+                      grads[k].numel() == C && grads[k].is_contiguous(),
+                  "bn_bwd_apply_cl: dgamma / dbeta must be [C] of x's dtype");
+    TORCH_CHECK(grads[2].scalar_type() == at::ScalarType::Float &&
+                    grads[2].numel() == parts * 2 * C &&
+                    grads[2].is_contiguous(),
+                "bn_bwd_apply_cl: local sums must be fp32 [parts, 2, C]");
+  }
   DISPATCH_FT(x, "bn_bwd_apply_cl", [&] {
     const bool wide = bn_wide(C, {raw_ptr(x), raw_ptr(dout), raw_ptr(dx)});
     bn_launch<scalar_t, kBnBwdApplyRows, kBnBwdApplyWide>(wide, [&](auto vc, auto rows) {
@@ -2884,9 +3081,33 @@
                          opt_ptr<scalar_t>(beta, has_affine),
                          sums.data_ptr<float>(), dx.data_ptr<scalar_t>(),
                          (int)C, M, 1.0f / (float)count, relu ? 1 : 0,
-                         has_affine ? 1 : 0, use_batch ? 1 : 0);
+                         has_affine ? 1 : 0, use_batch ? 1 : 0,
+                         opt_ptr<scalar_t>(with_grads ? grads[0] : x, with_grads),
+                         opt_ptr<scalar_t>(with_grads ? grads[1] : x, with_grads),
+                         with_grads ? grads[2].data_ptr<float>() : nullptr,
+                         (int)parts);
     });
   });
+}
+
+void bn_bwd_apply_cl(Tensor x, Tensor dout, Tensor mean,
+                     Tensor istd, Tensor gamma, Tensor beta,
+                     Tensor sums, Tensor dx,
+                     int64_t C, int64_t M, bool relu, bool has_affine,
+                     bool use_batch, int64_t parts, int64_t count) {
+  bn_bwd_apply_cl_impl(x, dout, mean, istd, gamma, beta, sums, dx, {}, C, M,
+                       relu, has_affine, use_batch, parts, count);
+}
+
+void bn_bwd_apply_cl_grads(Tensor x, Tensor dout, Tensor mean,
+                           Tensor istd, Tensor gamma, Tensor beta,
+                           Tensor sums, Tensor dx, Tensor dgamma, Tensor dbeta,
+                           Tensor local_sums,
+                           int64_t C, int64_t M, bool relu, bool has_affine,
+                           bool use_batch, int64_t parts, int64_t count) {
+  bn_bwd_apply_cl_impl(x, dout, mean, istd, gamma, beta, sums, dx,
+                       {dgamma, dbeta, local_sums}, C, M, relu, has_affine,
+                       use_batch, parts, count);
 }
 
 void matfn_chol_fwd(Tensor cov, Tensor W, Tensor L, double eps) {
@@ -2898,15 +3119,63 @@
                      L.data_ptr<float>(), g, (float)eps);
 }
 
+dwt::GdbOperand<float> gdb_flat(const Tensor& gdb) {
+  return {gdb.data_ptr<float>(), nullptr, nullptr, nullptr, nullptr, 0, 0};
+}
+
+template <typename F>
+void with_gdb_from_dgb(const char* name, const Tensor& W, const Tensor& dgb,
+                       const Tensor& gamma, const Tensor& dgamma,
+                       const Tensor& dbeta, bool has_affine, int64_t parts,
+                       F&& f) {
+  const int64_t n_groups = W.size(0), g = W.size(1);
+  TORCH_CHECK(parts >= 1 && (n_groups * g) % parts == 0, name, ": parts");
+  const int64_t C = n_groups * g / parts;
+  TORCH_CHECK(dgb.scalar_type() == at::ScalarType::Float &&
+                  dgb.is_contiguous() && dgb.numel() == parts * 2 * C,
+              name, ": dgb must be fp32 [parts, 2, C]");
+  if (!has_affine) {
+    f(dwt::GdbOperand<float>{nullptr, dgb.data_ptr<float>(), nullptr, nullptr,
+                             nullptr, (int)C, (int)parts});
+    return;
+  }
+  for (const Tensor* t : {&gamma, &dgamma, &dbeta})
+    TORCH_CHECK(t->scalar_type() == gamma.scalar_type() && t->numel() == C &&
+                    t->is_contiguous(),
+                name, ": gamma / dgamma / dbeta must be [C] of one dtype");
+  DISPATCH_FT(gamma, name, [&] {
+    f(dwt::GdbOperand<scalar_t>{nullptr, dgb.data_ptr<float>(),
+                                gamma.data_ptr<scalar_t>(),
+                                dgamma.data_ptr<scalar_t>(),
+                                dbeta.data_ptr<scalar_t>(), (int)C, (int)parts});
+  });
+}
+
+template <typename T>
+void launch_matfn_chol_bwd(Tensor dW, Tensor W, Tensor L,
+                           dwt::GdbOperand<T> gdb, Tensor S, Tensor corr,
+                           double eps, double inv_m) {
+  const int n_groups = W.size(0);
+  const int g = W.size(1);
+  hipLaunchKernelGGL(dwt::matfn_chol_bwd_kernel<T>, dim3(n_groups), dim3(64),
+                     0, cur_stream(), dW.data_ptr<float>(), W.data_ptr<float>(),
+                     L.data_ptr<float>(), gdb, S.data_ptr<float>(),
+                     corr.data_ptr<float>(), g, (float)eps, (float)inv_m);
+}
+
 void matfn_chol_bwd(Tensor dW, Tensor W, Tensor L, Tensor gdb, Tensor S,
                     Tensor corr, double eps, double inv_m) {
-  const int n_groups = W.size(0);
-  const int g = W.size(1);
-  hipLaunchKernelGGL(dwt::matfn_chol_bwd_kernel, dim3(n_groups), dim3(64), 0,
-                     cur_stream(), dW.data_ptr<float>(), W.data_ptr<float>(),
-                     L.data_ptr<float>(), gdb.data_ptr<float>(),
-                     S.data_ptr<float>(), corr.data_ptr<float>(), g, (float)eps,
-                     (float)inv_m);
+  launch_matfn_chol_bwd(dW, W, L, gdb_flat(gdb), S, corr, eps, inv_m);
+}
+
+void matfn_chol_bwd_dgb(Tensor dW, Tensor W, Tensor L, Tensor dgb,
+                        Tensor gamma, Tensor dgamma, Tensor dbeta, Tensor S,
+                        Tensor corr, double eps, double inv_m, bool has_affine,
+                        int64_t parts) {
+  with_gdb_from_dgb("matfn_chol_bwd", W, dgb, gamma, dgamma, dbeta, has_affine,
+                    parts, [&](auto gdb) {
+                      launch_matfn_chol_bwd(dW, W, L, gdb, S, corr, eps, inv_m);
+                    });
 }
 
 void matfn_ns_fwd(Tensor cov, Tensor W, Tensor ys, Tensor zs, Tensor svals,
@@ -2920,17 +3189,36 @@
                      svals.data_ptr<float>(), g, (float)eps, (int)iters);
 }
 
+template <typename T>
+void launch_matfn_ns_bwd(Tensor dW, Tensor W, Tensor ys, Tensor zs,
+                         Tensor svals, dwt::GdbOperand<T> gdb, Tensor S,
+                         Tensor corr, double eps, double inv_m, int64_t iters) {
+  const int n_groups = W.size(0);
+  const int g = W.size(1);
+  hipLaunchKernelGGL(dwt::matfn_ns_bwd_kernel<T>, dim3(n_groups), dim3(64), 0,
+                     cur_stream(), dW.data_ptr<float>(), W.data_ptr<float>(),
+                     ys.data_ptr<float>(), zs.data_ptr<float>(),
+                     svals.data_ptr<float>(), gdb, S.data_ptr<float>(),
+                     corr.data_ptr<float>(), g, (float)eps, (float)inv_m,
+                     (int)iters);
+}
+
 void matfn_ns_bwd(Tensor dW, Tensor W, Tensor ys, Tensor zs, Tensor svals,
                   Tensor gdb, Tensor S, Tensor corr, double eps, double inv_m,
                   int64_t iters) {
-  const int n_groups = W.size(0);
-  const int g = W.size(1);
-  hipLaunchKernelGGL(dwt::matfn_ns_bwd_kernel, dim3(n_groups), dim3(64), 0,
-                     cur_stream(), dW.data_ptr<float>(), W.data_ptr<float>(),
-                     ys.data_ptr<float>(), zs.data_ptr<float>(),
-                     svals.data_ptr<float>(), gdb.data_ptr<float>(),
-                     S.data_ptr<float>(), corr.data_ptr<float>(), g, (float)eps,
-                     (float)inv_m, (int)iters);
+  launch_matfn_ns_bwd(dW, W, ys, zs, svals, gdb_flat(gdb), S, corr, eps, inv_m,
+                      iters);
+}
+
+void matfn_ns_bwd_dgb(Tensor dW, Tensor W, Tensor ys, Tensor zs, Tensor svals,
+                      Tensor dgb, Tensor gamma, Tensor dgamma, Tensor dbeta,
+                      Tensor S, Tensor corr, double eps, double inv_m,
+                      int64_t iters, bool has_affine, int64_t parts) {
+  with_gdb_from_dgb("matfn_ns_bwd", W, dgb, gamma, dgamma, dbeta, has_affine,
+                    parts, [&](auto gdb) {
+                      launch_matfn_ns_bwd(dW, W, ys, zs, svals, gdb, S, corr,
+                                          eps, inv_m, iters);
+                    });
 }
 
 void maxpool_cl_fwd(Tensor x, Tensor out, Tensor idx, int64_t C, int64_t H,
@@ -3199,15 +3487,18 @@
   m.def("whiten_stats_partial", &whiten_stats_partial);
   m.def("whiten_stats_partial_cl", &whiten_stats_partial_cl);
   m.def("whiten_stats_final", &whiten_stats_final);
+  m.def("whiten_stats_final_ema", &whiten_stats_final_ema);
   m.def("bn_stats_partial", &bn_stats_partial);
   m.def("bn_stats_partial_cl", &bn_stats_partial_cl);
   m.def("bn_stats_final", &bn_stats_final);
+  m.def("bn_stats_final_ema", &bn_stats_final_ema);
   m.def("whiten_apply_cl", &whiten_apply_cl);
   m.def("whiten_bwd_reduce_cl", &whiten_bwd_reduce_cl);
   m.def("whiten_bwd_apply_cl", &whiten_bwd_apply_cl);
   m.def("bn_apply_cl", &bn_apply_cl);
   m.def("bn_bwd_reduce_cl", &bn_bwd_reduce_cl);
   m.def("bn_bwd_apply_cl", &bn_bwd_apply_cl);
+  m.def("bn_bwd_apply_cl", &bn_bwd_apply_cl_grads);
   m.def("whiten_apply_res_cl", &whiten_apply_res_cl);
   m.def("bn_apply_res_cl", &bn_apply_res_cl);
   m.def("whiten_join_bwd_reduce_cl", &whiten_join_bwd_reduce_cl);
@@ -3216,8 +3507,10 @@
   m.def("norm_wide_selected", &norm_wide_selected);
   m.def("matfn_chol_fwd", &matfn_chol_fwd);
   m.def("matfn_chol_bwd", &matfn_chol_bwd);
+  m.def("matfn_chol_bwd", &matfn_chol_bwd_dgb);
   m.def("matfn_ns_fwd", &matfn_ns_fwd);
   m.def("matfn_ns_bwd", &matfn_ns_bwd);
+  m.def("matfn_ns_bwd", &matfn_ns_bwd_dgb);
   m.def("whiten_apply", &whiten_apply);
   m.def("whiten_bwd_reduce", &whiten_bwd_reduce);
   m.def("whiten_bwd_apply", &whiten_bwd_apply);
diff --git a/dwt_amd/models/sites.py b/dwt_amd/models/sites.py
--- a/dwt_amd/models/sites.py
+++ b/dwt_amd/models/sites.py
@@ -53,7 +53,8 @@
 
     if isinstance(first, (_DomainBatchNorm, nn.modules.batchnorm._BatchNorm)):
         momentum = first.momentum if first.momentum is not None else 0.0
-        if training and first.track_running_stats:
+        counters = Fdwt.folded_counters(x, use, training)
+        if training and first.track_running_stats and counters is None:
             for b in use:
                 if b.num_batches_tracked is not None:
                     b.num_batches_tracked += 1
@@ -68,7 +69,7 @@
         kw = dict(parts=parts, eps=first.eps, momentum=momentum,
                   training=training,
                   track_running_stats=first.track_running_stats,
-                  stats_acc=stats_acc)
+                  stats_acc=stats_acc, counters=counters)
         if residual is not None:
             return Fdwt.norm_join("bn", x, residual, gamma, beta, rms, rvs, **kw)
         return Fdwt.batch_norm_multi(x, gamma, beta, rms, rvs, relu=relu, **kw)
diff --git a/dwt_amd/ops/batch_norm.py b/dwt_amd/ops/batch_norm.py
--- a/dwt_amd/ops/batch_norm.py
+++ b/dwt_amd/ops/batch_norm.py
@@ -62,7 +62,8 @@
 
     def _bn(self, x):
         momentum = self.momentum if self.momentum is not None else 0.0
-        if self.training and self.track_running_stats:
+        counters = Fdwt.folded_counters(x, [self], self.training)
+        if self.training and self.track_running_stats and counters is None:
             self.num_batches_tracked += 1
             if self.momentum is None:
                 momentum = 1.0 / self.num_batches_tracked.item()
@@ -82,7 +83,8 @@
             [self.running_mean] if self.track_running_stats else None,
             [self.running_var] if self.track_running_stats else None,
             parts=1, eps=self.eps, momentum=momentum, training=self.training,
-            relu=False, track_running_stats=self.track_running_stats)
+            relu=False, track_running_stats=self.track_running_stats,
+            counters=counters)
         return out.squeeze(-1) if squeeze else out
 
 
diff --git a/dwt_amd/ops/functional.py b/dwt_amd/ops/functional.py
--- a/dwt_amd/ops/functional.py
+++ b/dwt_amd/ops/functional.py
@@ -439,6 +439,7 @@
     relu: bool = False,
     track_running_stats: bool = True,
     stats_acc: Optional[torch.Tensor] = None,
+    counters: Optional[Sequence[torch.Tensor]] = None,
 ) -> torch.Tensor:
     cfg = _bn_cfg(parts=parts, eps=eps, momentum=momentum, training=training,
                   relu=relu, track_running_stats=track_running_stats)
@@ -446,8 +447,10 @@
         from ..kernels import dispatch
         if dispatch.available():
             return dispatch.batch_norm_multi(x, gamma, beta, running_means,
-                                             running_vars, cfg, stats_acc)
+                                             running_vars, cfg, stats_acc,
+                                             counters)
         dispatch.require_or_warn("batch_norm_multi")
+    assert counters is None, "counters are handed to the HIP forward only"
     return BatchNormMulti.apply(x, gamma, beta, running_means, running_vars, cfg)
 
 
@@ -565,6 +568,29 @@
     return AddReluFn.apply(a, b)
 
 
+def site_fold_enabled() -> bool:
+    return os.environ.get("DWT_AMD_SITE_FOLD", "1") != "0"
+
+
+def folded_counters(x: torch.Tensor, branches: Sequence[torch.nn.Module],
+                    training: bool):
+    first = branches[0]
+    if not (training and x.is_cuda and first.track_running_stats
+            and first.momentum is not None and site_fold_enabled()):
+        return None
+    from ..kernels import dispatch
+    if not dispatch.available():
+        return None
+    from ..kernels import hip_ops
+    counters = [b.num_batches_tracked for b in branches]
+    if hip_ops.bn_fold_takes_counters(
+            x, [b.running_mean for b in branches],
+            [b.running_var for b in branches], counters, len(branches),
+            training, True, first.momentum):
+        return counters
+    return None
+
+
 def fused_join_enabled() -> bool:
     return os.environ.get("DWT_AMD_FUSED_JOIN", "1") != "0"
 
@@ -582,6 +608,7 @@
     assert kind in ("whiten", "bn"), kind
     kw = dict(kw, relu=False)
     stats_acc = kw.pop("stats_acc", None)
+    counters = kw.pop("counters", None)
     if x.is_cuda and fused_join_enabled():
         from ..kernels import dispatch
         if dispatch.available():
@@ -591,8 +618,10 @@
                 fn = hip_ops.whiten_join if kind == "whiten" \
                     else hip_ops.batch_norm_join
                 return fn(x, identity, gamma, beta, running_means,
-                          running_vars, cfg, stats_acc)
+                          running_vars, cfg, stats_acc, counters)
     multi = whiten_multi if kind == "whiten" else batch_norm_multi
+    if counters is not None:
+        kw["counters"] = counters
     y = add_relu(multi(x, gamma, beta, running_means, running_vars,
                        stats_acc=stats_acc, **kw),
                  identity)
```

After: 9691 images/sec, median of 6. About the same (+0.7%).
